# rmazzier/OpenSetGaitRecognition_PCAA

Hardware: AMD Instinct MI355X
Metric: gait sequences/sec (train step) (higher is better)
Workload: dtype bf16; 1 GPU; PCAA V4 train step (enc+dec+disc fwd/bwd, WGAN-GP, Chamfer, 2x Adam), B=64/GPU T=30 N=128 C=4 K=8, BASELINE config[1]; global_batch=64, precision=bf16, parallelism=dp1, sync_bn=False, finite_loss=True, hip_graph=False, decoder_update=fused wgrad+adam

## Files before the change

include/pcaa_hip.h:

```cpp
#ifndef PCAA_HIP_H
#define PCAA_HIP_H

#include <stddef.h>

#ifdef __cplusplus
extern "C" {
#endif

#define PCAA_ABI_VERSION 20

#define PCAA_OK 0
#define PCAA_ERR_INVALID_ARG 1
#define PCAA_ERR_LAUNCH 2

#define PCAA_F32 0
#define PCAA_BF16 1
#define PCAA_SPLIT_F16 2

#define PCAA_LAYOUT_KC 0
#define PCAA_LAYOUT_RC 1

#define PCAA_ACT_NONE 0
#define PCAA_ACT_ELU 1

const char* pcaa_last_error(void);
int pcaa_abi_version(void);

int pcaa_gemm(int math,
              const void* A, int a_dtype, int a_layout, long lda,
              const void* B, int b_dtype, int b_layout, long ldb,
              void* C, int c_dtype, long ldc,
              int M, int N, int K,
              const float* bias, double* colstats, int nrep,
              int split_k, int accumulate, void* stream);

int pcaa_gemm_num_splits(int math, int K, int split_k);
int pcaa_gemm_group_rc_f32(int n, const void* const* A, const void* const* B, void* const* C, const int* M,
                           const int* N, const int* K, const int* split_k, void* stream);
int pcaa_gemm_group_rc_f32_slabs(int n, const void* const* A, const void* const* B, void* const* slabs, const int* M,
                                 const int* N, const int* K, const int* split_k, void* stream);
int pcaa_gemm_v2_enable(int on);
int pcaa_gemm_slabs(int math,
                    const void* A, int a_dtype, int a_layout, long lda,
                    const void* B, int b_dtype, int b_layout, long ldb,
                    float* slabs, long slab_stride, int M, int N, int K, int split_k, void* stream);
int pcaa_gemm_affine_elu(const void* A, long lda, const void* W, long ldw, void* out, long ldo,
                         const float* scale, const float* shift, int M, int N, int K, int pool_rows,
                         void* stream);
int pcaa_gemm_dgrad_bn_supported(int M, int N, int K);
int pcaa_gemm_dgrad_bn(const void* dy, long lddy, const void* Wt, long ldw, const void* y, void* dz, long ld,
                       const float* scale, const float* shift, const float* mean, const float* rstd,
                       double* stats, int nrep, int M, int N, int K,
                       const float* x, int xc, const float* W1, void* stream);
int pcaa_bn_bwd_dy_split(const float* dz, const float* y, void* dy_img, const float* coef, long rows, int ch,
                         float img_scale, void* stream);
int pcaa_gemm_dgrad_bn_split3(const void* dy_img, long lddy, const void* Wt_img, long ldw, const float* y, float* dz,
                              long ld, const float* scale, const float* shift, const float* mean, const float* rstd,
                              double* stats, int nrep, int M, int N, int K, float out_scale, void* stream);
int pcaa_timing_events_create(void** start, void** stop);
int pcaa_timing_events_destroy(void* start, void* stop);
int pcaa_time_next_gemm(void* start, void* stop);
int pcaa_timing_pending(void);
int pcaa_timing_elapsed_ms(void* start, void* stop, float* ms);
int pcaa_splitk_reduce(const float* slabs, int nsplit, long slab_stride, long n, float* out,
                       int accumulate, void* stream);
int pcaa_splitk_reduce_stats(const float* slabs, int nsplit, long slab_stride, float* out,
                             double* stats, int nrep, long rows, int ch, void* stream);

int pcaa_pointnet_in_fwd(const float* x, int C, const float* W, const float* bias, void* y, int y_dtype,
                         long P, int cout, double* stats, int nrep, void* stream);
int pcaa_pointnet_in_wgrad(const void* dy, int dy_dtype, const float* x, int C, float* dW, long P,
                           int cout, void* stream);
int pcaa_pointnet_in_apply(const float* x, int C, const float* W, const float* scale, const float* shift,
                           void* a, int a_dtype, long P, int cout, void* stream);
int pcaa_pointnet_in_bwd_stats(const void* da, int dtype, const float* x, int C, const float* W,
                               const float* scale, const float* shift, const float* mean, const float* rstd,
                               double* stats, int nrep, long P, int cout, void* stream);
int pcaa_pointnet_in_bwd_onepass(const void* da, int dtype, const float* x, int C, const float* W,
                                 const float* scale, const float* shift, const float* mean, const float* rstd,
                                 double* stats, int nrep, float* G, long P, int cout, const double* pivot_mom,
                                 double pivot_inv_count, void* stream);
int pcaa_pointnet_in_bwd_onepass_rows(const void* da, int dtype, const float* x, int C, const float* W,
                                      const float* scale, const float* shift, const float* mean, const float* rstd,
                                      double* stats, int nrep, float* G, long P, int cout, const double* pivot_mom,
                                      double pivot_inv_count, void* stream);
int pcaa_pointnet_in_bwd_g_rows(long P);
int pcaa_points_moments_size(void);
int pcaa_points_moments(const float* x, int C, long P, double* mom, void* stream);
int pcaa_pointnet_in_bwd_combine(const float* G, int nrep, const float* W, const double* mom, const float* coef,
                                 float* dW, int cout, int C, long P, const double* pivot_mom, double pivot_inv_count,
                                 void* stream);
int pcaa_pointnet_in_moment_stats(const double* mom, const float* W, int C, int cout, void* stream);
int pcaa_pointnet_in_bwd_wgrad(const void* da, int dtype, const float* x, int C, const float* W,
                               const float* scale, const float* shift, const float* coef, float* dW,
                               long P, int cout, int dz_is_pre ,
                               void* stream);

int pcaa_cast_bf16(const float* src, void* dst, void* dst_t, int R, int C, void* stream);

int pcaa_bn_finalize(const double* stats, int nrep, long count, const float* lin_bias,
                     const float* gamma, const float* beta,
                     float* running_mean, float* running_var, long long* num_batches_tracked,
                     float momentum, float eps,
                     float* scale, float* shift, float* mean, float* rstd, int ch, void* stream);
int pcaa_bn_eval_coeffs(const float* gamma, const float* beta, const float* running_mean,
                        const float* running_var, const float* lin_bias, float eps, float* scale,
                        float* shift, int ch, void* stream);
int pcaa_bn_act_fwd(const void* y, void* a, int dtype, const float* scale, const float* shift,
                    long rows, int ch, void* stream);
int pcaa_bn_act_meanpool_fwd(const void* y, int dtype, const float* scale, const float* shift,
                             const float* mean, const float* rstd, float* pooled, float* e1, float* e2,
                             long groups, int group_rows, int ch, void* stream);
int pcaa_bn_pool_bwd_stats(const float* dpool, const float* e1, const float* e2, float pool_scale,
                           double* stats, int nrep, long groups, int ch, void* stream);
int pcaa_bn_act_bwd_dz(const void* da, const float* dpool, int group_rows, float pool_scale,
                       const void* y, void* dz, int dtype,
                       const float* scale, const float* shift, const float* mean, const float* rstd,
                       double* stats, int nrep, long rows, int ch, void* stream);
int pcaa_bn_bwd_finalize(const double* stats, int nrep, long count, const float* gamma,
                         const float* mean, const float* rstd,
                         float* coef, float* dgamma, float* dbeta, int ch, void* stream);
int pcaa_bn_bwd_dy(const void* dz, const void* y, void* dy, int dtype, const float* coef,
                   long rows, int ch, void* stream);
int pcaa_bn_tail_arm_fwd(const double* stats, int nrep, long count, const float* lin_bias,
                         const float* gamma, const float* beta,
                         float* running_mean, float* running_var, long long* num_batches_tracked,
                         float momentum, float eps,
                         float* scale, float* shift, float* mean, float* rstd, int ch, unsigned* counter);
int pcaa_bn_tail_arm_bwd(const double* stats, int nrep, long count, const float* gamma,
                         const float* mean, const float* rstd,
                         float* coef, float* dgamma, float* dbeta, int ch, unsigned* counter);
int pcaa_bn_tail_pending(void);
int pcaa_bn_tail_disarm(void);
int pcaa_bn_bwd_dy_fused(const void* da, const float* dpool, int group_rows, float pool_scale,
                         const void* y, void* dy, int dtype, const float* scale, const float* shift,
                         const float* coef, long rows, int ch, void* stream);

int pcaa_bias_act(float* y, const float* bias, int act, long rows, int cols, void* stream);
int pcaa_elu_bwd_from_out(const float* da, const float* a, float* dz, long n, void* stream);
int pcaa_colsum(const float* x, float* out, long rows, int cols, void* stream);
int pcaa_sum(const float* x, long n, float scale, float* out, void* stream);
int pcaa_rowsum(const float* x, float* out, long rows, int cols, float scale, void* stream);
int pcaa_scale_by_device_scalar(const float* x, const float* s, float* out, long n, void* stream);
int pcaa_scale_rows(const float* x, const float* s, float* out, long rows, int cols, void* stream);
int pcaa_prior_sample(const float* z0, const float* means, const long long* gt, int B, int K, int D,
                      float* z, float* onehot, void* stream);
int pcaa_pack_points(const float* src, long sb, long sc, long st, long sn,
                     float* dst, int B, int C, int T, int N, void* stream);

int pcaa_gather_rows(const void* src, long n_src_rows, long row_bytes, const long long* idx, void* dst,
                     long n_rows, int* err_flag, void* stream);

int pcaa_dtc_im2col(const float* a, float* col, int B, int T, int Cin, int dilation, void* stream);
int pcaa_dtc_col2im(const float* dcol, float* da, int B, int T, int Cin, int dilation, void* stream);

int pcaa_chamfer_fwd_bwd(const float* preds, long p_sb, long p_sc, long p_st, long p_sn,
                         const float* gts, long g_sb, long g_sc, long g_st, long g_sn,
                         int B, int T, int N, int C, float* frame_loss,
                         float* dpreds, long d_sb, long d_sc, long d_st, long d_sn,
                         float grad_scale, const float* grad_per_b, void* stream);
int pcaa_cross_entropy(const float* logits, const long long* target, int B, int K,
                       float* loss, float* dlogits, float grad_scale, long long* preds,
                       int* err_flag, void* stream);

int pcaa_disc_forward(const float* x, const float* label, int B, int K,
                      const float* W1, const float* b1, const float* W2, const float* b2,
                      const float* W3, const float* b3, float* out, void* stream);
int pcaa_disc_backward(const float* x, const float* label, int B, int K,
                       const float* W1, const float* b1, const float* W2, const float* b2,
                       const float* W3, const float* b3, const float* gout,
                       float* dx, float* dlabel,
                       float* dW1, float* db1, float* dW2, float* db2, float* dW3, float* db3,
                       float* workspace, size_t workspace_bytes, void* stream);
int pcaa_disc_backward_backward(const float* x, const float* label, int B, int K,
                                const float* W1, const float* b1, const float* W2, const float* b2,
                                const float* W3, const float* b3, const float* gout, const float* gbar,
                                float* dx2, float* dlabel2, float* dgout,
                                float* dW1, float* db1, float* dW2, float* db2, float* dW3, float* db3,
                                float* workspace, size_t workspace_bytes, void* stream);
size_t pcaa_disc_workspace_bytes(int B, int K);
int pcaa_disc_wgan_gp(const float* z, const float* fv, const float* label, const float* alphas,
                      int B, int K,
                      const float* W1, const float* b1, const float* W2, const float* b2,
                      const float* W3, const float* b3, float gp_weight, float* losses,
                      float* dW1, float* db1, float* dW2, float* db2, float* dW3, float* db3,
                      float* dz, float* workspace, size_t workspace_bytes, void* stream);

int pcaa_joint_likelihood(const float* x, const float* means, int B, int K, int D, double* lik,
                          void* stream);
int pcaa_kvote(const double* lik, const long long* preds, double threshold, int k, int n_labels,
               int n_classes, int n_windows, long long* out, void* stream);

int pcaa_skinny_supported(int M, int N, int K);
int pcaa_skinny_splits(int kind, int M, int N, int K);
int pcaa_skinny_linear_fwd(const float* x, long ldx, const float* W, long ldw, const float* bias, int act,
                           float* y, float* ws, long ws_floats, int M, int N, int K, int nsplit,
                           void* stream);
int pcaa_skinny_linear_dgrad(const float* dz, long lddz, const float* W, long ldw, float* dx,
                             const float* a_prev, int accumulate, float* ws, long ws_floats, int M, int N,
                             int K, int nsplit, void* stream);
int pcaa_skinny_linear_wgrad(const float* dz, long lddz, const float* x, long ldx, float* dW, long lddw,
                             int M, int N, int K, void* stream);
int pcaa_skinny_linear_fwd_exact(const float* x, long ldx, const float* W, long ldw, const float* bias, int act,
                                 float* y, float* ws, long ws_floats, int M, int N, int K, int nsplit, void* stream);
int pcaa_skinny_linear_dgrad_exact(const float* dz, long lddz, const float* W, long ldw, float* dx,
                                   const float* a_prev, int accumulate, float* ws, long ws_floats, int M, int N,
                                   int K, int nsplit, void* stream);
int pcaa_skinny_linear_wgrad_exact(const float* dz, long lddz, const float* x, long ldx, float* dW, long lddw,
                                   int M, int N, int K, void* stream);
int pcaa_skinny_linear_wgrad_adam_exact(const float* dz, long lddz, const float* x, long ldx, float* W,
                                        float* exp_avg, float* exp_avg_sq, long ldw, int M, int N, int K,
                                        float beta1, float beta2, float eps, float grad_scale,
                                        const float* coef_dev, void* stream);
int pcaa_skinny_linear_wgrad_bf16(const float* dz, long lddz, const float* x, long ldx, void* dW_bf16, long lddw,
                                  int M, int N, int K, void* stream);
int pcaa_skinny_linear_wgrad_adam(const float* dz, long lddz, const float* x, long ldx, float* W,
                                  float* exp_avg, float* exp_avg_sq, long ldw, int M, int N, int K,
                                  float beta1, float beta2, float eps, float grad_scale,
                                  const float* coef_dev, void* stream);
int pcaa_skinny_linear_wgrad_adam_rows(const float* dz, long lddz, const float* x, long ldx, float* W,
                                       float* exp_avg, float* exp_avg_sq, long ldw, int M, int N, int K,
                                       float beta1, float beta2, float eps, float grad_scale,
                                       const float* coef_dev, int rows_alloc, void* stream);
long pcaa_packed_chunk_elems(int N, int K);
int pcaa_pack_rows_t16(const float* dz, long lddz, int N, const float* x, long ldx, int K, int rows, void* chunk_bf16,
                       void* stream);
int pcaa_skinny_linear_wgrad_adam_t16(const void* packed_bf16, long chunk_stride, int chunks, float* W, float* exp_avg,
                                      float* exp_avg_sq, long ldw, int N, int K, float beta1, float beta2, float eps,
                                      float grad_scale, const float* coef_dev, void* stream);
int pcaa_skinny_linear_fwd_w16(const float* x, long ldx, const void* W16, long ldw, const float* bias, int act,
                               float* y, float* ws, long ws_floats, int M, int N, int K, int nsplit, void* stream);
int pcaa_skinny_linear_dgrad_w16(const float* dz, long lddz, const void* W16, long ldw, float* dx,
                                 const float* a_prev, int accumulate, float* ws, long ws_floats, int M, int N,
                                 int K, int nsplit, void* stream);

int pcaa_dtc_conv_supported(int T, int cin, int cout);
int pcaa_dtc_conv_ksplit(int B, int cin, int cout);
int pcaa_dtc_conv_fwd(const float* src, const float* scale, const float* shift, const float* W, float* y,
                      float* col, double* stats, int nrep, int B, int T, int cin, int cout, int dilation,
                      int ksplit, long slab_stride, void* stream);
int pcaa_dtc_conv_fwd_bf16(const float* src, const float* scale, const float* shift, const float* W, float* y,
                      float* col, double* stats, int nrep, int B, int T, int cin, int cout, int dilation,
                      int ksplit, long slab_stride, void* stream);
// ... 4 lines not shown
                          void* stream);
int pcaa_dtc_conv_fwd_win_bf16(const float* table, const float* scale, const float* shift, const float* W, float* y,
                          float* col, double* stats, int nrep, int B, int T, int cin, int cout, int dilation,
                          int ksplit, long slab_stride, const int* win_row, long table_rows, long ring_rows,
                          void* stream);

int pcaa_dtc_conv_fwd_seg(const float* table, const float* scale, const float* shift, const float* W, float* y,
                          int B, int T, int cin, int cout, int dilation, int ksplit, long slab_stride,
                          const int* win_row, long n_seg, long ring_rows, void* stream);
int pcaa_dtc_conv_fwd_seg_bf16(const float* table, const float* scale, const float* shift, const float* W, float* y,
                          int B, int T, int cin, int cout, int dilation, int ksplit, long slab_stride,
                          const int* win_row, long n_seg, long ring_rows, void* stream);

int pcaa_crop_overlap_vec_bytes(const float* crops, long crop_elems, long frame_elems);
int pcaa_crop_overlap(const float* crops, long crop_elems, long frame_elems, int M, int T, int hop, int* same,
                      void* stream);
int pcaa_gather_rows_w4(const void* src, long n_src_rows, long row_words, const long long* idx, void* dst,
                        long n_rows, int* err_flag, void* stream);

int pcaa_scatter_rows(const void* src, const int* dst_row, long n_rows, long row_words, void* dst, long n_dst_rows,
                      int* err_flag, void* stream);
int pcaa_stream_score(const float* logits, const float* sup_fv, const float* means, const int* run_start, int n_runs,
                      const int* win_stream, const int* win_j, const int* vote_pos, int nw, int K, int D, int Kc,
                      double threshold, int k, int n_labels, int n_classes, double* hist_lik, long long* hist_pred,
                      int max_streams, long long* preds, double* lik, long long* votes, int n_votes, void* stream);

#define PCAA_RAW_MAX_CARD 1024
#define PCAA_RAW_MAX_POINTS 1024
int pcaa_frames_from_raw(const void* points, int points_f64, long P, const int* offsets, int n, const int* pick,
                         const int* frame_key, long seed, int N, int C, int standardize, int divide_by_std,
                         float* out, int n_out, int* pick_out, int* err_flag, void* stream);
int pcaa_dtc_conv_dgrad_ksplit(int B, int cin, int cout);
int pcaa_dtc_conv_dgrad(const float* dy, const float* dz, const float* y, const float* coef, float* dy_out,
                        const float* W, float* out, const float* ep_y, const float* ep_scale,
                        const float* ep_shift, const float* ep_mean, const float* ep_rstd, double* ep_stats,
                        int nrep, int B, int T, int cin, int cout, int dilation, int ksplit, long slab_stride,
                        void* stream);
int pcaa_dtc_conv_dgrad_bf16(const float* dy, const float* dz, const float* y, const float* coef, float* dy_out,
                        const float* W, float* out, const float* ep_y, const float* ep_scale,
                        const float* ep_shift, const float* ep_mean, const float* ep_rstd, double* ep_stats,
                        int nrep, int B, int T, int cin, int cout, int dilation, int ksplit, long slab_stride,
                        void* stream);

int pcaa_heads_supported(int B, int K, int d_in, int d_sup, int d_head, int d_proj, int backward);
int pcaa_heads_fwd(const float* x4, const float* W1, const float* b1, const float* Wh, const float* bh,
                   const float* W2, const float* b2, const float* Wg, const float* bg, float* sup_fv,
                   float* h, float* logits, float* hproj, int B, int K, void* stream);
int pcaa_heads_bwd(const float* x4, const float* sup_fv, const float* h, const float* logits,
                   const float* hproj, const float* W1, const float* Wh, const float* W2,
                   const float* Wg, const float* d_logits, const float* d_sup, const float* d_hproj,
                   float* dW1, float* db1, float* dWh, float* dbh, float* dW2, float* db2, float* dWg,
                   float* dbg, float* dx4, int B, int K, void* stream);

int pcaa_gemm_split3_supported(int M, int N, int K);
int pcaa_gemm_split3(const void* A, const void* B, int layout, long lda, long ldb, float* C, long ldc, int M,
                     int N, int K, double* colstats, int nrep, float out_scale, void* stream);
int pcaa_gemm_split3_num_splits(int K, int split_k);
int pcaa_gemm_slabs_split3(const void* A, const void* B, int layout, long lda, long ldb, float* slabs,
                           long slab_stride, int M, int N, int K, int split_k, float out_scale, void* stream);
int pcaa_split_f16(const float* src, void* dst_img, long rows, int ch, int transpose, float img_scale, void* stream);
int pcaa_set_range_flag(int* dev_flag);
int pcaa_bn_act_fwd_split(const float* y, void* a_img, const float* scale, const float* shift, long rows,
                          int ch, float img_scale, void* stream);
int pcaa_bn_bwd_dy_fused_split(const float* da, const float* dpool, int group_rows, float pool_scale,
                               const float* y, void* dy_img, const float* scale, const float* shift,
                               const float* coef, long rows, int ch, float img_scale, void* stream);

int pcaa_orced_heads_supported(int B, int K, int d_in, int d_lat);
int pcaa_orced_heads_fwd(const float* x4, const float* Wmu, const float* bmu, const float* Wlv, const float* blv,
                         const float* eps, const float* Wc, const float* bc, float* mu, float* logvar, float* sup_fv,
                         float* logits, int B, int K, int d_in, int d_lat, void* stream);
int pcaa_orced_heads_bwd(const float* x4, const float* eps, const float* logvar, const float* sup_fv,
                         const float* Wmu, const float* Wlv, const float* Wc, const float* d_logits,
                         const float* d_sup, const float* d_mu, const float* d_logvar, float* ws, float* dWmu,
                         float* dbmu, float* dWlv, float* dblv, float* dWc, float* dbc, float* dx4, int B, int K,
                         int d_in, int d_lat, void* stream);
int pcaa_orced_kl(const float* mu, const float* logvar, const float* mu_k, float* loss, float* d_mu,
                  float* d_logvar, float* d_muk, float gscale, int B, int d_lat, void* stream);

int pcaa_adam_step(float* param, const float* grad, float* exp_avg, float* exp_avg_sq, long n,
                   float lr, float beta1, float beta2, float eps, int step, float grad_scale,
                   int max_blocks, void* stream);
int pcaa_adam_advance(int* step_dev, float* coef_dev, float lr, float beta1, float beta2, void* stream);
int pcaa_adam_step_dev(float* param, const float* grad, float* exp_avg, float* exp_avg_sq, long n,
                       float beta1, float beta2, float eps, const float* coef_dev, float grad_scale,
                       int max_blocks, void* stream);
int pcaa_adam_step_dev_g16(float* param, const void* grad_bf16, float* exp_avg, float* exp_avg_sq, long n,
                           float beta1, float beta2, float eps, const float* coef_dev, float grad_scale,
                           int max_blocks, void* stream);

#ifdef __cplusplus
}
#endif
#endif
```

opensetgaitrecognition_pcaa_amd/csrc/elementwise.hip:

```cpp
#include <stdarg.h>

#include "common.h"
#include "bn_tail.h"

static thread_local char g_err[512] = "";
void pcaa_set_error(const char* fmt, ...) {
  va_list ap;
  va_start(ap, fmt);
  vsnprintf(g_err, sizeof(g_err), fmt, ap);
  va_end(ap);
}
extern "C" const char* pcaa_last_error(void) { return g_err; }
static thread_local int* g_range_flag = nullptr;
int* pcaa_range_flag_ptr() { return g_range_flag; }
extern "C" int pcaa_set_range_flag(int* dev_flag) { g_range_flag = dev_flag; return PCAA_OK; }
extern "C" int pcaa_abi_version(void) { return PCAA_ABI_VERSION; }

namespace {

constexpr int ROWS_PER_BLOCK = 128;

inline bool ch_ok(int ch) {
  if (ch < 4 || ch > 1024 || (ch & 3)) return false;
  const int q = ch >> 2;
// ... 455 lines not shown
    const int n = (int)(r % N); r /= N;
    const int t = (int)(r % T);
    const long b = r / T;
    dst[i] = src[b * sb + c * sc + t * st + n * sn];
  }
}

__global__ void dtc_im2col_kernel(const float* __restrict__ a, float* __restrict__ col, int B, int T,
                                  int Cin, int d) {
  const long total = (long)B * T * Cin * 3;
  for (long i = (long)blockIdx.x * blockDim.x + threadIdx.x; i < total; i += (long)gridDim.x * blockDim.x) {
    const int tap = (int)(i % 3);
    long r = i / 3;
    const int ci = (int)(r % Cin); r /= Cin;
    const int t = (int)(r % T);
    const long b = r / T;
    const int ts = t - (2 - tap) * d;
    col[i] = ts >= 0 ? a[(b * T + ts) * Cin + ci] : 0.f;
  }
}

__global__ void dtc_col2im_kernel(const float* __restrict__ dcol, float* __restrict__ da, int B, int T,
                                  int Cin, int d) {
  const long total = (long)B * T * Cin;
  for (long i = (long)blockIdx.x * blockDim.x + threadIdx.x; i < total; i += (long)gridDim.x * blockDim.x) {
    const int ci = (int)(i % Cin);
    long r = i / Cin;
    const int t = (int)(r % T);
    const long b = r / T;
    float acc = 0.f;
#pragma unroll
    for (int tap = 0; tap < 3; ++tap) {
      const int tt = t + (2 - tap) * d;
      if (tt < T) acc += dcol[((b * T + tt) * Cin + ci) * 3 + tap];
    }
    da[i] = acc;
  }
}

template <int U, typename TG = float>
__global__ __launch_bounds__(256) void adam_kernel(float* __restrict__ p, const TG* __restrict__ g,
                                                   float* __restrict__ m, float* __restrict__ v, long n,
                                                   float b1, float b2, float eps, float step_size,
                                                   float inv_bc2_sqrt, float grad_scale,
                                                   const float* __restrict__ coef) {
  if (coef) {
    step_size = coef[0];
    inv_bc2_sqrt = coef[1];
  }
  const long nq = n >> 2;
  const long stride = (long)gridDim.x * 256;
  for (long q0 = (long)blockIdx.x * 256 + threadIdx.x; q0 < nq; q0 += stride * U) {
    f32x4 pv[U], gv[U], mv[U], vv[U];
#pragma unroll
    for (int u = 0; u < U; ++u) {
      const long q = q0 + u * stride;
      if (q < nq) { pv[u] = load4(p + q * 4); gv[u] = load4(g + q * 4); mv[u] = load4(m + q * 4); vv[u] = load4(v + q * 4); }
    }
#pragma unroll
    for (int u = 0; u < U; ++u) {
      const long q = q0 + u * stride;
      if (q >= nq) break;
#pragma unroll
      for (int e = 0; e < 4; ++e) {
        float pe = pv[u][e], me = mv[u][e], ve = vv[u][e];
        adam_update(pe, me, ve, gv[u][e] * grad_scale, b1, b2, eps, step_size, inv_bc2_sqrt);
        pv[u][e] = pe; mv[u][e] = me; vv[u][e] = ve;
      }
      store4(p + q * 4, pv[u]);
      store4(m + q * 4, mv[u]);
      store4(v + q * 4, vv[u]);
    }
  }
  if (blockIdx.x == 0 && threadIdx.x < (n & 3)) {
    const long i = (nq << 2) + threadIdx.x;
    float pp = p[i], mm = m[i], vv = v[i];
    adam_update(pp, mm, vv, (float)g[i] * grad_scale, b1, b2, eps, step_size, inv_bc2_sqrt);
    m[i] = mm;
    v[i] = vv;
    p[i] = pp;
  }
}

__global__ void adam_coef_kernel(int* __restrict__ step, float* __restrict__ coef, float lr, float b1, float b2) {
  const int t = *step + 1;
  *step = t;
  const double bc1 = 1.0 - pow((double)b1, (double)t);
  const double bc2 = 1.0 - pow((double)b2, (double)t);
  coef[0] = (float)((double)lr / bc1);
  coef[1] = (float)(1.0 / sqrt(bc2));
}

inline int grid_for(long work_items, int per_block = 256, int cap = 256 * 8) {
  long g = cdiv(work_items, per_block);
  if (g < 1) g = 1;
  if (g > cap) g = cap;
  return (int)g;
}

inline int col_invariant_grid(long nquads, int qpr) {
  int a = qpr, b = 256;
  while (b) { const int t = a % b; a = b; b = t; }
  const int unit = qpr / a;
  long g = cdiv(nquads, 256);
  if (g > 2048) g = 2048;
  g = cdiv(g, unit) * unit;
  return (int)g;
}

}

extern "C" int pcaa_bn_finalize(const double* stats, int nrep, long count, const float* lin_bias,
                                const float* gamma, const float* beta, float* running_mean,
                                float* running_var, long long* num_batches_tracked, float momentum,
                                float eps, float* scale, float* shift, float* mean, float* rstd,
                                int ch, void* stream) {
  PCAA_CHECK_ARG(stats && gamma && beta && scale && shift && mean && rstd, "pcaa_bn_finalize: null pointer");
  PCAA_CHECK_ARG(nrep >= 1 && count >= 1 && ch >= 1, "pcaa_bn_finalize: bad sizes");
  PCAA_CHECK_ARG((running_mean == nullptr) == (running_var == nullptr), "pcaa_bn_finalize: running stats must come together");
  const double unbias = count > 1 ? (double)count / (double)(count - 1) : 1.0;
  hipLaunchKernelGGL(bn_finalize_kernel, dim3((unsigned)cdiv(ch, 256)), dim3(256), 0, as_stream(stream),
                     stats, nrep, 1.0 / (double)count, unbias, lin_bias, gamma, beta, running_mean,
                     running_var, num_batches_tracked, momentum, eps, scale, shift, mean, rstd, ch);
  PCAA_RETURN_LAUNCH_STATUS("pcaa_bn_finalize");
}

extern "C" int pcaa_bn_eval_coeffs(const float* gamma, const float* beta, const float* running_mean,
                                   const float* running_var, const float* lin_bias, float eps, float* scale,
                                   float* shift, int ch, void* stream) {
  PCAA_CHECK_ARG(gamma && beta && running_mean && running_var && scale && shift && ch >= 1, "pcaa_bn_eval_coeffs: bad args");
  hipLaunchKernelGGL(bn_eval_coeffs_kernel, dim3((unsigned)cdiv(ch, 256)), dim3(256), 0, as_stream(stream),
                     gamma, beta, running_mean, running_var, lin_bias, eps, scale, shift, ch);
  PCAA_RETURN_LAUNCH_STATUS("pcaa_bn_eval_coeffs");
}

extern "C" int pcaa_bn_act_fwd(const void* y, void* a, int dtype, const float* scale, const float* shift,
                               long rows, int ch, void* stream) {
  PCAA_CHECK_ARG(y && a && scale && shift, "pcaa_bn_act_fwd: null pointer");
  PCAA_CHECK_ARG(rows >= 1 && ch >= 4 && (ch & 3) == 0, "pcaa_bn_act_fwd: ch must be a multiple of 4");
  const long nq = rows * (ch >> 2);
  PCAA_CHECK_ARG(nq < (1L << 31), "pcaa_bn_act_fwd: tensor too large for 32-bit quad indices");
  const int grid = col_invariant_grid(nq, ch >> 2);
  if (dtype == PCAA_F32)
    hipLaunchKernelGGL(bn_act_fwd_kernel<float>, dim3(grid), dim3(256), 0, as_stream(stream),
                       (const float*)y, (float*)a, scale, shift, (unsigned)nq, (unsigned)(ch >> 2));
  else if (dtype == PCAA_BF16)
    hipLaunchKernelGGL(bn_act_fwd_kernel<bf16_t>, dim3(grid), dim3(256), 0, as_stream(stream),
                       (const bf16_t*)y, (bf16_t*)a, scale, shift, (unsigned)nq, (unsigned)(ch >> 2));
  else { pcaa_set_error("pcaa_bn_act_fwd: bad dtype"); return PCAA_ERR_INVALID_ARG; }
  PCAA_RETURN_LAUNCH_STATUS("pcaa_bn_act_fwd");
}

extern "C" int pcaa_bn_act_fwd_split(const float* y, void* a_img, const float* scale, const float* shift, long rows,
                                     int ch, float img_scale, void* stream) {
  PCAA_CHECK_ARG(y && a_img && scale && shift, "pcaa_bn_act_fwd_split: null pointer");
  PCAA_CHECK_ARG(rows >= 1 && ch >= 4 && (ch & 3) == 0, "pcaa_bn_act_fwd_split: ch must be a multiple of 4");
  const long nq = rows * (ch >> 2);
  PCAA_CHECK_ARG(nq < (1L << 31), "pcaa_bn_act_fwd_split: tensor too large for 32-bit quad indices");
  const int grid = col_invariant_grid(nq, ch >> 2);
  hipLaunchKernelGGL(bn_act_fwd_split_kernel, dim3(grid), dim3(256), 0, as_stream(stream), y, (split_t*)a_img, scale, shift,
                     (unsigned)nq, (unsigned)(ch >> 2), img_scale, pcaa_range_flag_ptr());
  PCAA_RETURN_LAUNCH_STATUS("pcaa_bn_act_fwd_split");
}

extern "C" int pcaa_split_f16(const float* src, void* dst_img, long rows, int ch, int transpose, float img_scale,
                               void* stream) {
  PCAA_CHECK_ARG(src && dst_img && rows >= 1 && ch >= 1, "pcaa_split_f16: bad args");
  long g = cdiv(rows * ch, 256);
  if (g > 4096) g = 4096;
  hipLaunchKernelGGL(split_f16_kernel, dim3((unsigned)g), dim3(256), 0, as_stream(stream), src, (split_t*)dst_img, rows, ch,
                     transpose, img_scale, pcaa_range_flag_ptr());
  PCAA_RETURN_LAUNCH_STATUS("pcaa_split_f16");
}
// ... 303 lines not shown
  const int n = B * (D > K ? D : K);
  hipLaunchKernelGGL(prior_sample_kernel, dim3((unsigned)cdiv(n, 256)), dim3(256), 0, as_stream(stream), z0, means, gt, B, K, D, z, onehot);
  PCAA_RETURN_LAUNCH_STATUS("pcaa_prior_sample");
}

extern "C" int pcaa_pack_points(const float* src, long sb, long sc, long st, long sn, float* dst,
                                int B, int C, int T, int N, void* stream) {
  PCAA_CHECK_ARG(src && dst && B >= 1 && C >= 1 && T >= 1 && N >= 1, "pcaa_pack_points: bad args");
  const long n = (long)B * C * T * N;
  hipLaunchKernelGGL(pack_points_kernel, dim3(grid_for(n)), dim3(256), 0, as_stream(stream), src, sb, sc, st, sn, dst, B, C, T, N);
  PCAA_RETURN_LAUNCH_STATUS("pcaa_pack_points");
}

namespace {
__global__ __launch_bounds__(256) void gather_rows_kernel(const uint4* __restrict__ src, const long long* __restrict__ idx,
                                                          long n_src, uint4* __restrict__ dst, long n_rows,
                                                          long row_vec, int* __restrict__ err) {
  const long total = n_rows * row_vec;
  for (long v = (long)blockIdx.x * 256 + threadIdx.x; v < total; v += (long)gridDim.x * 256) {
    const long r = v / row_vec, off = v - r * row_vec;
    const long long i = idx[r];
    uint4 val = {0u, 0u, 0u, 0u};
    if (i >= 0 && i < n_src) val = src[i * row_vec + off];
    else if (err != nullptr && off == 0) atomicOr(err, 1);
    dst[v] = val;
  }
}
}

extern "C" int pcaa_gather_rows(const void* src, long n_src_rows, long row_bytes, const long long* idx, void* dst,
                                long n_rows, int* err_flag, void* stream) {
  PCAA_CHECK_ARG(src && idx && dst && n_src_rows >= 1 && n_rows >= 1 && row_bytes >= 16 && row_bytes % 16 == 0,
                 "pcaa_gather_rows: bad args (rows are multiples of 16 bytes)");
  PCAA_CHECK_ARG(((uintptr_t)src % 16) == 0 && ((uintptr_t)dst % 16) == 0, "pcaa_gather_rows: 16-B alignment");
  const long row_vec = row_bytes / 16;
  hipLaunchKernelGGL(gather_rows_kernel, dim3(grid_for(n_rows * row_vec, 256, 256 * 16)), dim3(256), 0, as_stream(stream),
                     reinterpret_cast<const uint4*>(src), idx, n_src_rows, reinterpret_cast<uint4*>(dst), n_rows,
                     row_vec, err_flag);
  PCAA_RETURN_LAUNCH_STATUS("pcaa_gather_rows");
}

extern "C" int pcaa_dtc_im2col(const float* a, float* col, int B, int T, int Cin, int dilation, void* stream) {
  PCAA_CHECK_ARG(a && col && B >= 1 && T >= 1 && Cin >= 1 && dilation >= 1, "pcaa_dtc_im2col: bad args");
  const long n = (long)B * T * Cin * 3;
  hipLaunchKernelGGL(dtc_im2col_kernel, dim3(grid_for(n)), dim3(256), 0, as_stream(stream), a, col, B, T, Cin, dilation);
  PCAA_RETURN_LAUNCH_STATUS("pcaa_dtc_im2col");
}

extern "C" int pcaa_dtc_col2im(const float* dcol, float* da, int B, int T, int Cin, int dilation, void* stream) {
  PCAA_CHECK_ARG(dcol && da && B >= 1 && T >= 1 && Cin >= 1 && dilation >= 1, "pcaa_dtc_col2im: bad args");
  const long n = (long)B * T * Cin;
  hipLaunchKernelGGL(dtc_col2im_kernel, dim3(grid_for(n)), dim3(256), 0, as_stream(stream), dcol, da, B, T, Cin, dilation);
  PCAA_RETURN_LAUNCH_STATUS("pcaa_dtc_col2im");
}

namespace {
__device__ __forceinline__ void slab_sum(const float* __restrict__ base, int nsplit, long stride, f32x4& acc) {
  int s = 0;
  for (; s + 8 <= nsplit; s += 8) {
    f32x4 v[8];
#pragma unroll
    for (int u = 0; u < 8; ++u) v[u] = load4(base + (s + u) * stride);
#pragma unroll
    for (int u = 0; u < 8; ++u) acc += v[u];
  }
  for (; s < nsplit; ++s) acc += load4(base + s * stride);
}

__global__ __launch_bounds__(256) void splitk_reduce_kernel(const float* __restrict__ slabs, int nsplit,
                                                            long stride, long nquads, float* __restrict__ out,
                                                            int accumulate) {
  for (long q = (long)blockIdx.x * 256 + threadIdx.x; q < nquads; q += (long)gridDim.x * 256) {
    f32x4 acc = accumulate ? load4(out + q * 4) : f32x4{0.f, 0.f, 0.f, 0.f};
    slab_sum(slabs + q * 4, nsplit, stride, acc);
    store4(out + q * 4, acc);
  }
}
}

namespace {
__global__ __launch_bounds__(256) void splitk_reduce_stats_kernel(const float* __restrict__ slabs, int nsplit,
                                                                  long stride, float* __restrict__ out,
                                                                  double* __restrict__ stats, int nrep,
                                                                  long rows, int ch) {
  __shared__ f32x4 red[2][256];
  const int qpr = ch >> 2, rl = 256 / qpr;
  const int cq = threadIdx.x % qpr, rlane = threadIdx.x / qpr;
  const int c = cq * 4;
  constexpr int RPB = 32;
  const long r0 = (long)blockIdx.x * RPB, r1 = min(rows, r0 + RPB);
  f32x4 s1 = {0.f, 0.f, 0.f, 0.f}, s2 = {0.f, 0.f, 0.f, 0.f};
  for (long r = r0 + rlane; r < r1; r += rl) {
    f32x4 acc = {0.f, 0.f, 0.f, 0.f};
    slab_sum(slabs + r * ch + c, nsplit, stride, acc);
    store4(out + r * ch + c, acc);
    s1 += acc;
    s2 += acc * acc;
  }
  red[0][threadIdx.x] = s1;
  red[1][threadIdx.x] = s2;
  __syncthreads();
  for (int o = threadIdx.x; o < 2 * ch; o += 256) {
    const int stat = o / ch, cc = o - stat * ch;
    double v = 0.0;
    for (int l = 0; l < rl; ++l) v += (double)red[stat][l * qpr + (cc >> 2)][cc & 3];
    unsafeAtomicAdd(&stats[((long)(blockIdx.x % nrep) * 2 + stat) * ch + cc], v);
  }
}
}

extern "C" int pcaa_splitk_reduce_stats(const float* slabs, int nsplit, long slab_stride, float* out,
                                        double* stats, int nrep, long rows, int ch, void* stream) {
  PCAA_CHECK_ARG(slabs && out && stats && nsplit >= 1 && nrep >= 1 && rows >= 1, "pcaa_splitk_reduce_stats: bad args");
  PCAA_CHECK_ARG(ch_ok(ch) && (slab_stride % 4) == 0, "pcaa_splitk_reduce_stats: ch/4 must divide 256 (ch=%d)", ch);
  hipLaunchKernelGGL(splitk_reduce_stats_kernel, dim3((unsigned)cdiv(rows, 32)), dim3(256), 0, as_stream(stream),
                     slabs, nsplit, slab_stride, out, stats, nrep, rows, ch);
  PCAA_RETURN_LAUNCH_STATUS("pcaa_splitk_reduce_stats");
}

extern "C" int pcaa_splitk_reduce(const float* slabs, int nsplit, long slab_stride, long n, float* out,
                                  int accumulate, void* stream) {
  PCAA_CHECK_ARG(slabs && out && nsplit >= 1 && n >= 4 && (n % 4) == 0 && (slab_stride % 4) == 0,
                 "pcaa_splitk_reduce: n and slab_stride must be multiples of 4");
  PCAA_CHECK_ARG(((uintptr_t)slabs % 16) == 0 && ((uintptr_t)out % 16) == 0, "pcaa_splitk_reduce: 16-B alignment");
  hipLaunchKernelGGL(splitk_reduce_kernel, dim3(grid_for(n >> 2)), dim3(256), 0, as_stream(stream), slabs, nsplit,
                     slab_stride, n >> 2, out, accumulate);
  PCAA_RETURN_LAUNCH_STATUS("pcaa_splitk_reduce");
}

static int launch_adam(float* param, const float* grad, float* exp_avg, float* exp_avg_sq, long n, float beta1,
                       float beta2, float eps, float step_size, float inv_bc2_sqrt, const float* coef,
                       float grad_scale, int max_blocks, void* stream, const char* what) {
  PCAA_CHECK_ARG(((uintptr_t)param % 16) == 0 && ((uintptr_t)grad % 16) == 0 && ((uintptr_t)exp_avg % 16) == 0 &&
                 ((uintptr_t)exp_avg_sq % 16) == 0, "pcaa_adam_step: buffers must be 16-B aligned");
  const int cap = max_blocks > 0 ? max_blocks : 256 * 16;
  if (cap <= 1024)
    hipLaunchKernelGGL(adam_kernel<4>, dim3(grid_for(n >> 4, 256, cap)), dim3(256), 0, as_stream(stream), param, grad,
                       exp_avg, exp_avg_sq, n, beta1, beta2, eps, step_size, inv_bc2_sqrt, grad_scale, coef);
  else
    hipLaunchKernelGGL(adam_kernel<1>, dim3(grid_for(n >> 2, 256, cap)), dim3(256), 0, as_stream(stream), param, grad,
                       exp_avg, exp_avg_sq, n, beta1, beta2, eps, step_size, inv_bc2_sqrt, grad_scale, coef);
  PCAA_RETURN_LAUNCH_STATUS(what);
}

extern "C" int pcaa_adam_step_dev_g16(float* param, const void* grad_bf16, float* exp_avg, float* exp_avg_sq, long n,
                                      float beta1, float beta2, float eps, const float* coef_dev, float grad_scale,
                                      int max_blocks, void* stream) {
  PCAA_CHECK_ARG(param && grad_bf16 && exp_avg && exp_avg_sq && coef_dev && n >= 1 && max_blocks >= 0,
                 "pcaa_adam_step_dev_g16: bad args");
  PCAA_CHECK_ARG(((uintptr_t)param % 16) == 0 && ((uintptr_t)grad_bf16 % 8) == 0 && ((uintptr_t)exp_avg % 16) == 0 &&
                 ((uintptr_t)exp_avg_sq % 16) == 0, "pcaa_adam_step_dev_g16: buffers must be 16-B (gradient: 8-B) aligned");
  const bf16_t* g = reinterpret_cast<const bf16_t*>(grad_bf16);
  const int cap = max_blocks > 0 ? max_blocks : 256 * 16;
  if (cap <= 1024)
    hipLaunchKernelGGL((adam_kernel<4, bf16_t>), dim3(grid_for(n >> 4, 256, cap)), dim3(256), 0, as_stream(stream), param, g,
                       exp_avg, exp_avg_sq, n, beta1, beta2, eps, 0.f, 0.f, grad_scale, coef_dev);
  else
    hipLaunchKernelGGL((adam_kernel<1, bf16_t>), dim3(grid_for(n >> 2, 256, cap)), dim3(256), 0, as_stream(stream), param, g,
                       exp_avg, exp_avg_sq, n, beta1, beta2, eps, 0.f, 0.f, grad_scale, coef_dev);
  PCAA_RETURN_LAUNCH_STATUS("pcaa_adam_step_dev_g16");
}

extern "C" int pcaa_adam_step(float* param, const float* grad, float* exp_avg, float* exp_avg_sq, long n,
                              float lr, float beta1, float beta2, float eps, int step, float grad_scale,
                              int max_blocks, void* stream) {
  PCAA_CHECK_ARG(param && grad && exp_avg && exp_avg_sq && n >= 1 && step >= 1 && max_blocks >= 0,
                 "pcaa_adam_step: bad args");
  const double bc1 = 1.0 - pow((double)beta1, (double)step);
  const double bc2 = 1.0 - pow((double)beta2, (double)step);
  return launch_adam(param, grad, exp_avg, exp_avg_sq, n, beta1, beta2, eps, (float)((double)lr / bc1),
                     (float)(1.0 / sqrt(bc2)), nullptr, grad_scale, max_blocks, stream, "pcaa_adam_step");
}

extern "C" int pcaa_adam_advance(int* step_dev, float* coef_dev, float lr, float beta1, float beta2, void* stream) {
  PCAA_CHECK_ARG(step_dev && coef_dev, "pcaa_adam_advance: bad args");
  hipLaunchKernelGGL(adam_coef_kernel, dim3(1), dim3(1), 0, as_stream(stream), step_dev, coef_dev, lr, beta1, beta2);
  PCAA_RETURN_LAUNCH_STATUS("pcaa_adam_advance");
}

extern "C" int pcaa_adam_step_dev(float* param, const float* grad, float* exp_avg, float* exp_avg_sq, long n,
                                  float beta1, float beta2, float eps, const float* coef_dev, float grad_scale,
                                  int max_blocks, void* stream) {
  PCAA_CHECK_ARG(param && grad && exp_avg && exp_avg_sq && coef_dev && n >= 1 && max_blocks >= 0,
                 "pcaa_adam_step_dev: bad args");
  return launch_adam(param, grad, exp_avg, exp_avg_sq, n, beta1, beta2, eps, 0.f, 0.f, coef_dev, grad_scale,
                     max_blocks, stream, "pcaa_adam_step_dev");
}
```

opensetgaitrecognition_pcaa_amd/csrc/losses.hip:

```cpp
#include "common.h"

namespace {

constexpr int MAXC = 8;
constexpr int CH_THREADS = 256;

__global__ __launch_bounds__(CH_THREADS) void chamfer_kernel(
    const float* __restrict__ preds, long p_sb, long p_sc, long p_st, long p_sn,
    const float* __restrict__ gts, long g_sb, long g_sc, long g_st, long g_sn,
    int T, int N, int C, float* __restrict__ frame_loss,
    float* __restrict__ dpreds, long d_sb, long d_sc, long d_st, long d_sn,
    float grad_scale, const float* __restrict__ grad_per_b) {
  extern __shared__ __attribute__((aligned(16))) float sm[];
  float* sg = sm;
  float* sp = sg + (long)N * MAXC;
  float* rg = sp + (long)N * MAXC;
  float* rp = rg + N;
  int* nn = reinterpret_cast<int*>(rp + N);
  __shared__ float red[CH_THREADS / 64];

  const int frame = blockIdx.x;
  const int b = frame / T, t = frame - b * T;
  const float* pb = preds + b * p_sb + t * p_st;
  const float* gb = gts + b * g_sb + t * g_st;

  for (int e = threadIdx.x; e < N * MAXC; e += CH_THREADS) {
    const int n = e / MAXC, c = e - n * MAXC;
    sg[e] = (c < C) ? gb[c * g_sc + n * g_sn] : 0.f;
    sp[e] = (c < C) ? pb[c * p_sc + n * p_sn] : 0.f;
  }
  __syncthreads();
  for (int n = threadIdx.x; n < N; n += CH_THREADS) {
    float a = 0.f, q = 0.f;
#pragma unroll
    for (int c = 0; c < MAXC; ++c) {
      a = fmaf(sg[n * MAXC + c], sg[n * MAXC + c], a);
      q = fmaf(sp[n * MAXC + c], sp[n * MAXC + c], q);
    }
    rg[n] = a;
    rp[n] = q;
  }
  __syncthreads();

  const float w = grad_scale * (grad_per_b ? grad_per_b[b] : 1.f);
  float loss = 0.f;
  for (int item = threadIdx.x; item < 2 * N; item += CH_THREADS) {
    const bool dir1 = item < N;
    const int me = dir1 ? item : item - N;
    const float* mine = dir1 ? sp : sg;
    const float* other = dir1 ? sg : sp;
    const float* rother = dir1 ? rg : rp;
    float v[MAXC];
#pragma unroll
    for (int c = 0; c < MAXC; ++c) v[c] = mine[me * MAXC + c];
    const float rme = dir1 ? rp[me] : rg[me];
    float best = 3.4e38f;
    int bi = 0;
    for (int o = 0; o < N; ++o) {
      float dot = 0.f;
#pragma unroll
      for (int c = 0; c < MAXC; ++c) dot = fmaf(other[o * MAXC + c], v[c], dot);
      const float P = (dir1 ? (rother[o] + rme) : (rme + rother[o])) - 2.f * dot;
      if (P < best) { best = P; bi = o; }
    }
    loss += best;
    nn[item] = bi;
  }
  loss = wave_sum(loss);
  if ((threadIdx.x & 63) == 0) red[threadIdx.x >> 6] = loss;
  __syncthreads();
  if (threadIdx.x == 0) {
    float tot = 0.f;
    for (int i = 0; i < CH_THREADS / 64; ++i) tot += red[i];
    frame_loss[frame] = tot;
  }
  if (dpreds) {
    __syncthreads();
    float* db = dpreds + b * d_sb + t * d_st;
    for (int e = threadIdx.x; e < N * C; e += CH_THREADS) {
      const int c = e / N, n = e - c * N;
      const float pv = sp[n * MAXC + c];
      float g = 2.f * w * (pv - sg[nn[n] * MAXC + c]);
      for (int i = 0; i < N; ++i)
        if (nn[N + i] == n) g += 2.f * w * (pv - sg[i * MAXC + c]);
      db[c * d_sc + n * d_sn] = g;
    }
  }
}

__global__ __launch_bounds__(256) void cross_entropy_kernel(const float* __restrict__ logits,
                                                            const long long* __restrict__ target, int B,
                                                            int K, float* loss, float* dlogits,
                                                            float grad_scale, long long* preds, int* err_flag) {
  __shared__ double red[4];
  double acc = 0.0;
  for (int r = threadIdx.x; r < B; r += 256) {
    const float* x = logits + (long)r * K;
    float mx = x[0];
    for (int k = 1; k < K; ++k) mx = fmaxf(mx, x[k]);
    float se = 0.f;
    for (int k = 0; k < K; ++k) se += expf(x[k] - mx);
    const float inv = 1.f / se;
    int am = 0;
    float pbest = -1.f;
    long long tg = target ? target[r] : 0;
    if (tg < 0 || tg >= K) {
      if (err_flag) *err_flag = 1;
      tg = 0;
    }
    for (int k = 0; k < K; ++k) {
      const float pk = expf(x[k] - mx) / se;
      if (pk > pbest) { pbest = pk; am = k; }
      if (dlogits) dlogits[(long)r * K + k] = grad_scale * (expf(x[k] - mx) * inv - (k == tg ? 1.f : 0.f)) / (float)B;
    }
    if (preds) preds[r] = am;
    if (target) acc += (double)(logf(se) + mx - x[tg]);
  }
  acc = wave_sum_d(acc);
  if ((threadIdx.x & 63) == 0) red[threadIdx.x >> 6] = acc;
  __syncthreads();
  if (threadIdx.x == 0 && loss) loss[0] = (float)((red[0] + red[1] + red[2] + red[3]) / B);
}

}

extern "C" int pcaa_chamfer_fwd_bwd(const float* preds, long p_sb, long p_sc, long p_st, long p_sn,
                                    const float* gts, long g_sb, long g_sc, long g_st, long g_sn,
                                    int B, int T, int N, int C, float* frame_loss, float* dpreds,
                                    long d_sb, long d_sc, long d_st, long d_sn, float grad_scale,
                                    const float* grad_per_b, void* stream) {
  PCAA_CHECK_ARG(preds && gts && frame_loss, "pcaa_chamfer_fwd_bwd: null pointer");
  PCAA_CHECK_ARG(B >= 1 && T >= 1 && N >= 1 && C >= 1 && C <= MAXC, "pcaa_chamfer_fwd_bwd: need 1<=C<=%d (C=%d)", MAXC, C);
  const size_t lds = ((size_t)2 * N * MAXC + 4 * (size_t)N) * sizeof(float);
  PCAA_CHECK_ARG(lds <= 150 * 1024, "pcaa_chamfer_fwd_bwd: N=%d too large for one LDS tile", N);
  if (lds > 64 * 1024) {
    hipError_t e = hipFuncSetAttribute(reinterpret_cast<const void*>(chamfer_kernel),
                                       hipFuncAttributeMaxDynamicSharedMemorySize, (int)lds);
    if (e != hipSuccess) { pcaa_set_error("pcaa_chamfer_fwd_bwd: cannot raise LDS limit: %s", hipGetErrorString(e)); return PCAA_ERR_LAUNCH; }
  }
  hipLaunchKernelGGL(chamfer_kernel, dim3((unsigned)(B * T)), dim3(CH_THREADS), lds, as_stream(stream),
                     preds, p_sb, p_sc, p_st, p_sn, gts, g_sb, g_sc, g_st, g_sn, T, N, C, frame_loss,
                     dpreds, d_sb, d_sc, d_st, d_sn, grad_scale, grad_per_b);
  PCAA_RETURN_LAUNCH_STATUS("pcaa_chamfer_fwd_bwd");
}

extern "C" int pcaa_cross_entropy(const float* logits, const long long* target, int B, int K, float* loss,
                                  float* dlogits, float grad_scale, long long* preds, int* err_flag,
                                  void* stream) {
  PCAA_CHECK_ARG(logits && B >= 1 && K >= 1, "pcaa_cross_entropy: bad args");
  PCAA_CHECK_ARG(target || (!loss && !dlogits), "pcaa_cross_entropy: loss/grad need targets");
  hipLaunchKernelGGL(cross_entropy_kernel, dim3(1), dim3(256), 0, as_stream(stream), logits, target, B, K,
                     loss, dlogits, grad_scale, preds, err_flag);
  PCAA_RETURN_LAUNCH_STATUS("pcaa_cross_entropy");
}
```

opensetgaitrecognition_pcaa_amd/csrc/pointnet_in.hip:

```cpp
#include "common.h"
#include "bn_tail.h"

namespace {

constexpr int MAXC = 8;
constexpr int FWD_ROWS = 128;
constexpr int WG_ROWS = 256;
constexpr int BWD_ROWS = 256;

template <typename T, int CP>
__global__ __launch_bounds__(256) void pointnet_in_fwd_kernel(const float* __restrict__ x, int C,
                                                              const float* __restrict__ W,
                                                              const float* __restrict__ bias,
                                                              T* __restrict__ y, long P, int cout,
                                                              double* __restrict__ stats, int nrep, BnTail tail) {
  __shared__ float xs[FWD_ROWS * CP];
  __shared__ f32x4 red[2][256];
  __shared__ int tail_flag;
  typedef float f32x2 __attribute__((ext_vector_type(2)));
  const int qpr = cout >> 2, rl = 256 / qpr;
  const int cq = threadIdx.x % qpr, rlane = threadIdx.x / qpr;
  const long r0 = (long)blockIdx.x * FWD_ROWS;
  const int nrows = (int)min((long)FWD_ROWS, P - r0);
  for (int e = threadIdx.x; e < FWD_ROWS * CP; e += 256) {
// ... 269 lines not shown
    if (MODE == 3) __syncthreads();
  }
  if (MODE != 0) {
    float* red = xs;
#pragma unroll
    for (int j = 0; j < 4; ++j)
#pragma unroll
      for (int c = 0; c < CP; ++c) red[(rlane * cout + cq * 4 + j) * CP + c] = acc[j][c];
    __syncthreads();
    for (int o = threadIdx.x; o < cout * C; o += 256) {
      const int ch = o / C, c = o - ch * C;
      float v = 0.f;
      for (int l = 0; l < rl; ++l) v += red[(l * cout + ch) * CP + c];
      if (MODE == 3 && g_row_per_wg) dW[(long)blockIdx.x * cout * C + o] = v;
      else atomicAdd(&dW[(MODE == 3 ? (long)(blockIdx.x % nrep) * cout * C : 0L) + o], v);
    }
  }
  if (MODE == 0 || MODE == 3) bn_tail_run(tail, threadIdx.x, 256, gridDim.x, &tail_flag);
}

template <int CP>
__global__ __launch_bounds__(256) void points_moments_kernel(const float* __restrict__ x, int C, long P,
                                                             double* __restrict__ mom) {
  constexpr int NV = CP * (CP + 1) / 2 + CP;
  __shared__ double red[4][NV];
  double a[NV];
#pragma unroll
  for (int i = 0; i < NV; ++i) a[i] = 0.0;
  for (long r = (long)blockIdx.x * 256 + threadIdx.x; r < P; r += (long)gridDim.x * 256) {
    double xv[CP];
    if (CP == 4 && C == 4) {
      const f32x4 v = load4(x + r * 4);
      xv[0] = v.x; xv[1] = v.y; xv[2] = v.z; xv[3] = v.w;
    } else {
#pragma unroll
      for (int c = 0; c < CP; ++c) xv[c] = c < C ? (double)x[r * C + c] : 0.0;
    }
    int i = 0;
#pragma unroll
    for (int k = 0; k < CP; ++k)
#pragma unroll
      for (int c = k; c < CP; ++c) { a[i] = fma(xv[k], xv[c], a[i]); ++i; }
#pragma unroll
    for (int c = 0; c < CP; ++c) a[i + c] += xv[c];
  }
#pragma unroll
  for (int i = 0; i < NV; ++i) {
    const double v = wave_sum_d(a[i]);
    if ((threadIdx.x & 63) == 0) red[threadIdx.x >> 6][i] = v;
  }
  __syncthreads();
  if (threadIdx.x < NV) {
    const double v = red[0][threadIdx.x] + red[1][threadIdx.x] + red[2][threadIdx.x] + red[3][threadIdx.x];
    int i = threadIdx.x;
    if (i < CP * (CP + 1) / 2) {
      int k = 0;
      while (i >= CP - k) { i -= CP - k; ++k; }
      const int c = k + i;
      unsafeAtomicAdd(&mom[k * MAXC + c], v);
      if (c != k) unsafeAtomicAdd(&mom[c * MAXC + k], v);
    } else {
      unsafeAtomicAdd(&mom[MAXC * MAXC + (i - CP * (CP + 1) / 2)], v);
    }
  }
}

__global__ void pointnet_in_moment_stats_kernel(const double* __restrict__ mom, const float* __restrict__ W, int C,
                                                BnTail t) {
  const int o = blockIdx.x * blockDim.x + threadIdx.x;
  if (o == 0 && t.kind == 1 && t.nbt != nullptr) *t.nbt += 1;
  if (o >= t.ch) return;
  double w[MAXC];
  for (int k = 0; k < MAXC; ++k) w[k] = k < C ? (double)W[o * C + k] : 0.0;
  double s1 = 0.0, s2 = 0.0;
  for (int k = 0; k < C; ++k) {
    s1 += w[k] * mom[MAXC * MAXC + k];
    double row = 0.0;
    for (int c = 0; c < C; ++c) row += mom[k * MAXC + c] * w[c];
    s2 += w[k] * row;
  }
  bn_tail_channel(t, o, s1, s2);
}

__global__ __launch_bounds__(256) void pointnet_in_bwd_combine_kernel(const float* __restrict__ G, int g_rows,
                                                                      const float* __restrict__ W,
                                                                      const double* __restrict__ mom,
                                                                      const float* __restrict__ coef,
                                                                      float* __restrict__ dW, int cout, int C, double P,
                                                                      const double* __restrict__ pivot_mom,
                                                                      double pivot_inv_count) {
  __shared__ double red[4];
  const int i = blockIdx.x;
  const int o = i / C, c = i - o * C;
  double g = 0.0;
  for (int r = threadIdx.x; r < g_rows; r += 256) g += (double)G[(long)r * cout * C + i];
  g = wave_sum_d(g);
  if ((threadIdx.x & 63) == 0) red[threadIdx.x >> 6] = g;
  __syncthreads();
  if (threadIdx.x != 0) return;
  g = (red[0] + red[1]) + (red[2] + red[3]);
  const double piv = pivot_mom ? (double)(float)(pivot_mom[MAXC * MAXC + c] * pivot_inv_count) : 0.0;
  double yx = 0.0;
  for (int k = 0; k < C; ++k) yx += (double)W[o * C + k] * (mom[k * MAXC + c] - piv * mom[MAXC * MAXC + k]);
  dW[i] = (float)((double)coef[o] * g + (double)coef[cout + o] * yx +
                  (double)coef[2 * cout + o] * (mom[MAXC * MAXC + c] - P * piv));
}

template <typename T>
__global__ __launch_bounds__(256) void pointnet_in_wgrad_kernel(const T* __restrict__ dy,
                                                                const float* __restrict__ x, int C,
                                                                float* __restrict__ dW, long P, int cout) {
  __shared__ float xs[(WG_ROWS * MAXC > 8192) ? WG_ROWS * MAXC : 8192];
  const int qpr = cout >> 2, rl = 256 / qpr;
  const int cq = threadIdx.x % qpr, rlane = threadIdx.x / qpr;
  const long r0 = (long)blockIdx.x * WG_ROWS;
  const int nrows = (int)min((long)WG_ROWS, P - r0);
  for (int e = threadIdx.x; e < WG_ROWS * MAXC; e += 256) {
    const int r = e / MAXC, c = e - r * MAXC;
    xs[e] = (r < nrows && c < C) ? x[(r0 + r) * C + c] : 0.f;
  }
  __syncthreads();
  float acc[4][MAXC];
#pragma unroll
  for (int j = 0; j < 4; ++j)
#pragma unroll
    for (int c = 0; c < MAXC; ++c) acc[j][c] = 0.f;
  int r = rlane;
  for (; r + 3 * rl < nrows; r += 4 * rl) {
    f32x4 d[4];
#pragma unroll
    for (int u = 0; u < 4; ++u) d[u] = load4(dy + (r0 + r + u * rl) * cout + cq * 4);
#pragma unroll
    for (int u = 0; u < 4; ++u) {
#pragma unroll
      for (int c = 0; c < MAXC; ++c) {
        const float xv = xs[(r + u * rl) * MAXC + c];
        acc[0][c] = fmaf(d[u].x, xv, acc[0][c]);
        acc[1][c] = fmaf(d[u].y, xv, acc[1][c]);
        acc[2][c] = fmaf(d[u].z, xv, acc[2][c]);
        acc[3][c] = fmaf(d[u].w, xv, acc[3][c]);
      }
    }
  }
  for (; r < nrows; r += rl) {
    const f32x4 d = load4(dy + (r0 + r) * cout + cq * 4);
#pragma unroll
    for (int c = 0; c < MAXC; ++c) {
      const float xv = xs[r * MAXC + c];
      acc[0][c] = fmaf(d.x, xv, acc[0][c]);
      acc[1][c] = fmaf(d.y, xv, acc[1][c]);
      acc[2][c] = fmaf(d.z, xv, acc[2][c]);
      acc[3][c] = fmaf(d.w, xv, acc[3][c]);
    }
  }
  __syncthreads();
  float* red = xs;
#pragma unroll
  for (int j = 0; j < 4; ++j)
#pragma unroll
    for (int c = 0; c < MAXC; ++c) red[(rlane * cout + cq * 4 + j) * MAXC + c] = acc[j][c];
  __syncthreads();
  for (int o = threadIdx.x; o < cout * C; o += 256) {
    const int ch = o / C, c = o - ch * C;
    float v = 0.f;
    for (int l = 0; l < rl; ++l) v += red[(l * cout + ch) * MAXC + c];
    atomicAdd(&dW[o], v);
// ... 87 lines not shown
extern "C" int pcaa_pointnet_in_bwd_stats(const void* da, int dtype, const float* x, int C, const float* W,
                                          const float* scale, const float* shift, const float* mean,
                                          const float* rstd, double* stats, int nrep, long P, int cout,
                                          void* stream) {
  PCAA_CHECK_ARG(da && x && W && scale && shift && mean && rstd && stats && P >= 1 && nrep >= 1,
                 "pcaa_pointnet_in_bwd_stats: bad args");
  PCAA_CHECK_ARG(shape_ok(C, cout), "pcaa_pointnet_in_bwd_stats: need C<=%d and cout/4 dividing 256 (C=%d cout=%d)", MAXC, C, cout);
  const unsigned grid = (unsigned)cdiv(P, BWD_ROWS);
  const BnTail tail = pcaa_take_bn_tail(stats);
  if (dtype == PCAA_F32)
    LAUNCH_BWD(float, 0, (const float*)da, x, C, W, scale, shift, mean, rstd, nullptr, stats, nrep, nullptr, P, cout, tail);
  else if (dtype == PCAA_BF16)
    LAUNCH_BWD(bf16_t, 0, (const bf16_t*)da, x, C, W, scale, shift, mean, rstd, nullptr, stats, nrep, nullptr, P, cout, tail);
  else { pcaa_set_error("pcaa_pointnet_in_bwd_stats: bad dtype"); return PCAA_ERR_INVALID_ARG; }
  PCAA_RETURN_LAUNCH_STATUS("pcaa_pointnet_in_bwd_stats");
}

extern "C" int pcaa_pointnet_in_bwd_wgrad(const void* da, int dtype, const float* x, int C, const float* W,
                                          const float* scale, const float* shift, const float* coef, float* dW,
                                          long P, int cout, int dz_is_pre, void* stream) {
  PCAA_CHECK_ARG(da && x && W && scale && shift && coef && dW && P >= 1, "pcaa_pointnet_in_bwd_wgrad: bad args");
  PCAA_CHECK_ARG(shape_ok(C, cout), "pcaa_pointnet_in_bwd_wgrad: need C<=%d and cout/4 dividing 256 (C=%d cout=%d)", MAXC, C, cout);
  const unsigned grid = (unsigned)cdiv(P, BWD_ROWS);
  if (dtype == PCAA_F32 && !dz_is_pre)
    LAUNCH_BWD(float, 1, (const float*)da, x, C, W, scale, shift, nullptr, nullptr, coef, nullptr, 1, dW, P, cout, BnTail{});
  else if (dtype == PCAA_F32)
    LAUNCH_BWD(float, 2, (const float*)da, x, C, W, scale, shift, nullptr, nullptr, coef, nullptr, 1, dW, P, cout, BnTail{});
  else if (dtype == PCAA_BF16 && !dz_is_pre)
    LAUNCH_BWD(bf16_t, 1, (const bf16_t*)da, x, C, W, scale, shift, nullptr, nullptr, coef, nullptr, 1, dW, P, cout, BnTail{});
  else if (dtype == PCAA_BF16)
    LAUNCH_BWD(bf16_t, 2, (const bf16_t*)da, x, C, W, scale, shift, nullptr, nullptr, coef, nullptr, 1, dW, P, cout, BnTail{});
  else { pcaa_set_error("pcaa_pointnet_in_bwd_wgrad: bad dtype"); return PCAA_ERR_INVALID_ARG; }
  PCAA_RETURN_LAUNCH_STATUS("pcaa_pointnet_in_bwd_wgrad");
}

static int pointnet_in_bwd_onepass(const void* da, int dtype, const float* x, int C, const float* W, const float* scale,
                                   const float* shift, const float* mean, const float* rstd, double* stats, int nrep,
                                   float* G, long P, int cout, const double* pivot_mom, double pivot_inv_count,
                                   int g_row_per_wg, void* stream) {
  PCAA_CHECK_ARG(da && x && W && scale && shift && mean && rstd && stats && G && P >= 1 && nrep >= 1,
                 "pcaa_pointnet_in_bwd_onepass: bad args");
  PCAA_CHECK_ARG(shape_ok(C, cout), "pcaa_pointnet_in_bwd_onepass: need C<=%d and cout/4 dividing 256 (C=%d cout=%d)", MAXC, C, cout);
  const unsigned grid = (unsigned)cdiv(P, BWD_ROWS);
  const BnTail tail = pcaa_take_bn_tail(stats);
  if (dtype == PCAA_F32)
    LAUNCH_BWD(float, 3, (const float*)da, x, C, W, scale, shift, mean, rstd, nullptr, stats, nrep, G, P, cout, tail,
               pivot_mom, pivot_inv_count, g_row_per_wg);
  else if (dtype == PCAA_BF16)
    LAUNCH_BWD(bf16_t, 3, (const bf16_t*)da, x, C, W, scale, shift, mean, rstd, nullptr, stats, nrep, G, P, cout, tail,
               pivot_mom, pivot_inv_count, g_row_per_wg);
  else { pcaa_set_error("pcaa_pointnet_in_bwd_onepass: bad dtype"); return PCAA_ERR_INVALID_ARG; }
  PCAA_RETURN_LAUNCH_STATUS("pcaa_pointnet_in_bwd_onepass");
}

extern "C" int pcaa_pointnet_in_bwd_onepass(const void* da, int dtype, const float* x, int C, const float* W,
                                            const float* scale, const float* shift, const float* mean,
                                            const float* rstd, double* stats, int nrep, float* G, long P, int cout,
                                            const double* pivot_mom, double pivot_inv_count, void* stream) {
  return pointnet_in_bwd_onepass(da, dtype, x, C, W, scale, shift, mean, rstd, stats, nrep, G, P, cout, pivot_mom,
                                 pivot_inv_count, 0, stream);
}

extern "C" int pcaa_pointnet_in_bwd_onepass_rows(const void* da, int dtype, const float* x, int C, const float* W,
                                                 const float* scale, const float* shift, const float* mean,
                                                 const float* rstd, double* stats, int nrep, float* G, long P, int cout,
                                                 const double* pivot_mom, double pivot_inv_count, void* stream) {
  return pointnet_in_bwd_onepass(da, dtype, x, C, W, scale, shift, mean, rstd, stats, nrep, G, P, cout, pivot_mom,
                                 pivot_inv_count, 1, stream);
}

extern "C" int pcaa_pointnet_in_bwd_g_rows(long P) { return (int)cdiv(P, BWD_ROWS); }

extern "C" int pcaa_points_moments_size(void) { return MAXC * MAXC + MAXC; }

extern "C" int pcaa_points_moments(const float* x, int C, long P, double* mom, void* stream) {
  PCAA_CHECK_ARG(x && mom && C >= 1 && C <= MAXC && P >= 1, "pcaa_points_moments: bad args");
  long g = cdiv(P, 256 * 4);
  if (g > 512) g = 512;
  if (C <= 4) hipLaunchKernelGGL(points_moments_kernel<4>, dim3((unsigned)g), dim3(256), 0, as_stream(stream), x, C, P, mom);
  else hipLaunchKernelGGL(points_moments_kernel<8>, dim3((unsigned)g), dim3(256), 0, as_stream(stream), x, C, P, mom);
  PCAA_RETURN_LAUNCH_STATUS("pcaa_points_moments");
}

extern "C" int pcaa_pointnet_in_moment_stats(const double* mom, const float* W, int C, int cout, void* stream) {
  PCAA_CHECK_ARG(mom && W && C >= 1 && C <= MAXC && cout >= 1, "pcaa_pointnet_in_moment_stats: bad args");
  const BnTail t = pcaa_take_bn_tail(mom);
  PCAA_CHECK_ARG(t.kind == 1 && t.ch == cout, "pcaa_pointnet_in_moment_stats: arm the forward finalize on `mom` first "
                 "(pcaa_bn_tail_arm_fwd)");
  hipLaunchKernelGGL(pointnet_in_moment_stats_kernel, dim3((unsigned)cdiv(cout, 256)), dim3(256), 0, as_stream(stream), mom,
                     W, C, t);
  PCAA_RETURN_LAUNCH_STATUS("pcaa_pointnet_in_moment_stats");
}

extern "C" int pcaa_pointnet_in_bwd_combine(const float* G, int nrep, const float* W, const double* mom,
                                            const float* coef, float* dW, int cout, int C, long P,
                                            const double* pivot_mom, double pivot_inv_count, void* stream) {
  PCAA_CHECK_ARG(G && W && mom && coef && dW && cout >= 1 && C >= 1 && C <= MAXC && nrep >= 1,
                 "pcaa_pointnet_in_bwd_combine: bad args");
  hipLaunchKernelGGL(pointnet_in_bwd_combine_kernel, dim3((unsigned)(cout * C)), dim3(256), 0,
                     as_stream(stream), G, nrep, W, mom, coef, dW, cout, C, (double)P, pivot_mom, pivot_inv_count);
  PCAA_RETURN_LAUNCH_STATUS("pcaa_pointnet_in_bwd_combine");
}

extern "C" int pcaa_cast_bf16(const float* src, void* dst, void* dst_t, int R, int C, void* stream) {
  PCAA_CHECK_ARG(src && (dst || dst_t) && R >= 1 && C >= 1, "pcaa_cast_bf16: bad args");
  const long n = (long)R * C;
  long g = cdiv(n, 256);
  if (g > 2048) g = 2048;
  hipLaunchKernelGGL(cast_bf16_kernel, dim3((unsigned)g), dim3(256), 0, as_stream(stream), src, (bf16_t*)dst,
                     (bf16_t*)dst_t, R, C);
  PCAA_RETURN_LAUNCH_STATUS("pcaa_cast_bf16");
}
```

opensetgaitrecognition_pcaa_amd/ops.py:

```python
import ctypes
import os

import torch

from . import _lib
from ._lib import ACT_ELU, ACT_NONE, KC, PCAA_BF16, PCAA_F32, RC, check

PCAA_SPLIT_F16 = 2

NREP = 16
BN_EPS = 1e-5
BN_MOMENTUM = 0.1


def _p(t):
    return None if t is None else t.data_ptr()


_raw_stream = getattr(torch._C, "_cuda_getCurrentRawStream", None)
_raw_device = getattr(torch._C, "_cuda_getDevice", None)


def _s():
    if _raw_stream is not None and _raw_device is not None:
# ... 70 lines not shown
        return self.only_prefix is None or key.startswith(self.only_prefix)

    def summary(self):
        torch.cuda.synchronize()
        agg = {}
        for key, flops, nbytes, ev in self.records:
            if not ev.valid():
                continue
            a = agg.setdefault(key, {"launches": 0, "ms": 0.0, "flops": 0.0, "bytes": 0.0})
            a["launches"] += 1
            a["ms"] += ev.elapsed_ms()
            a["flops"] += flops
            a["bytes"] += nbytes
        return agg


class _TorchEvents:

    def __init__(self):
        self.e0 = torch.cuda.Event(enable_timing=True)
        self.e1 = torch.cuda.Event(enable_timing=True)
        self.e0.record()

    def end(self):
        self.e1.record()
        return self

    def valid(self):
        return True

    def elapsed_ms(self):
        return self.e0.elapsed_time(self.e1)


class _KernelEvents:

    def __init__(self):
        lib = _lib.load()
        self.a, self.b = ctypes.c_void_p(), ctypes.c_void_p()
        check(lib.pcaa_timing_events_create(ctypes.byref(self.a), ctypes.byref(self.b)), "pcaa_timing_events_create")
        check(lib.pcaa_time_next_gemm(self.a, self.b), "pcaa_time_next_gemm")
        self.ok = False

    def end(self):
        lib = _lib.load()
        self.ok = not lib.pcaa_timing_pending()
        if not self.ok:
            lib.pcaa_time_next_gemm(None, None)
        return self

    def valid(self):
        return self.ok

    def elapsed_ms(self):
        ms = ctypes.c_float()
        check(_lib.load().pcaa_timing_elapsed_ms(self.a, self.b, ctypes.byref(ms)), "pcaa_timing_elapsed_ms")
        return float(ms.value)

    def __del__(self):
        try:
            _lib.load().pcaa_timing_events_destroy(self.a, self.b)
        except Exception:
            pass


def _begin_timing(key):
    return _KernelEvents() if key.startswith(("gemm_bf16_v2_kernel", "gemm_bf16_v2rc_kernel")) else _TorchEvents()


TIMER = None


def set_timer(timer):
    global TIMER
    TIMER = timer


class StatsPool:

    def __init__(self, device, capacity_doubles=4 << 20):
        self.buf = torch.zeros(capacity_doubles, dtype=torch.float64, device=device)
        self.off = 0

    def begin(self):
        if self.off:
            self.buf[:self.off].zero_()
        self.off = 0

    def take_raw(self, n):
        n = (n + 1) // 2 * 2
        if self.off + n > self.buf.numel():
            return None
        v = self.buf[self.off:self.off + n]
        self.off += n
        return v

    def take(self, ch):
        n = NREP * 2 * ch
        if self.off + n + 2 > self.buf.numel():
            return None
        v = self.buf[self.off:self.off + n].view(NREP, 2, ch)
        v._pcaa_counter = self.buf[self.off + n:self.off + n + 1].view(torch.int32)
        self.off += n + 2
        return v


STATS_POOL = None


def set_stats_pool(pool):
    global STATS_POOL
    STATS_POOL = pool


def new_stats(ch, device):
    if STATS_POOL is not None and STATS_POOL.buf.device == torch.device(device):
        v = STATS_POOL.take(ch)
        if v is not None:
            return v
    buf = torch.zeros(NREP * 2 * ch + 2, dtype=torch.float64, device=device)
    v = buf[:NREP * 2 * ch].view(NREP, 2, ch)
    v._pcaa_counter = buf[NREP * 2 * ch:NREP * 2 * ch + 1].view(torch.int32)
    return v


TAILS = {"enabled": os.environ.get("PCAA_BN_TAIL", "1") != "0", "taken": 0, "standalone": 0}


class BnTailFwd:
    def __init__(self, count, lin_bias, bn, ch, sync=None, update_running=True):
        self.count, self.lin_bias, self.bn, self.ch, self.sync, self.update_running = count, lin_bias, bn, ch, sync, update_running
        self.out = None
        self.armed = False
        self.count_out = count

    def arm(self, stats):
        counter = getattr(stats, "_pcaa_counter", None)
        if self.sync is not None or counter is None or not TAILS["enabled"]:
            return
        dev, bn, ch = stats.device, self.bn, self.ch
        scale = torch.empty(ch, dtype=torch.float32, device=dev)
        self.out = (scale, torch.empty_like(scale), torch.empty_like(scale), torch.empty_like(scale))
        rm = bn.running_mean if self.update_running else None
        rv = bn.running_var if self.update_running else None
        nbt = bn.num_batches_tracked if self.update_running else None
        check(_lib.load().pcaa_bn_tail_arm_fwd(_p(stats), NREP, int(self.count), _p(self.lin_bias), _p(bn.weight), _p(bn.bias),
                                               _p(rm), _p(rv), _p(nbt), BN_MOMENTUM if bn.momentum is None else bn.momentum,
                                               bn.eps, *(_p(t) for t in self.out), ch, _p(counter)), "pcaa_bn_tail_arm_fwd")
        self.armed = True

    def resolve(self, stats):
        lib = _lib.load()
        if self.armed and not lib.pcaa_bn_tail_pending():
            TAILS["taken"] += 1
            return self.out
        if self.armed:
            lib.pcaa_bn_tail_disarm()
        count = self.sync(stats, self.count) if self.sync is not None else self.count
        self.count_out = count
        TAILS["standalone"] += 1
        self.out = bn_finalize(stats, count, self.lin_bias, self.bn, self.ch, self.update_running)
        return self.out


class BnTailBwd:
    def __init__(self, count, bn, mean, rstd, ch, dgamma=None, dbeta=None, sync=None):
        self.count, self.bn, self.mean, self.rstd, self.ch, self.sync = count, bn, mean, rstd, ch, sync
        self.dgamma, self.dbeta = dgamma, dbeta
        self.out = None
        self.armed = False
# ... 450 lines not shown
    return max(1, min(s, K // (4 * bk) if K >= 4 * bk else 1))


def cast_bf16(W2d, want_plain=True, want_transposed=True, out=None):
    _chk(W2d, "cast_bf16.W", torch.float32, 2)
    R, C = W2d.shape
    if out is not None:
        _chk(out, "cast_bf16.out", torch.bfloat16, 2)
        if tuple(out.shape) != (R, C):
            raise ValueError("cast_bf16: out shape")
    w = out if out is not None else (torch.empty((R, C), dtype=torch.bfloat16, device=W2d.device) if want_plain else None)
    wt = torch.empty((C, R), dtype=torch.bfloat16, device=W2d.device) if want_transposed else None
    check(_lib.load().pcaa_cast_bf16(_p(W2d), _p(w), _p(wt), R, C, _s()), "pcaa_cast_bf16")
    return w, wt


def pointnet_in_ok(C, cout):
    return 1 <= C <= 8 and cout % 4 == 0 and cout <= 1024 and 256 % (cout // 4) == 0


def pointnet_in_fwd(x2d, W2d, bias, out_dtype, stats=None, tail=None):
    _chk(x2d, "pointnet_in.x", torch.float32, 2)
    _chk(W2d, "pointnet_in.W", torch.float32, 2)
    P, C = x2d.shape
    cout = W2d.shape[0]
    if W2d.shape[1] != C or not pointnet_in_ok(C, cout):
        raise ValueError(f"pointnet_in_fwd: unsupported shape C={C} cout={cout}")
    if out_dtype is None:
        if stats is None:
            raise ValueError("pointnet_in_fwd: statistics-only call needs stats")
        if tail is not None:
            tail.arm(stats)
        check(_lib.load().pcaa_pointnet_in_fwd(_p(x2d), C, _p(W2d), None, None, PCAA_F32, P, cout, _p(stats), NREP,
                                               _s()), "pcaa_pointnet_in_fwd(stats)")
        if tail is not None:
            tail.resolve(stats)
        return None
    y = torch.empty((P, cout), dtype=out_dtype, device=x2d.device)
    if tail is not None and stats is not None:
        tail.arm(stats)
    check(_lib.load().pcaa_pointnet_in_fwd(_p(x2d), C, _p(W2d), _p(bias), _p(y), _dt(y), P, cout, _p(stats), NREP, _s()),
          "pcaa_pointnet_in_fwd")
    if tail is not None and stats is not None:
        tail.resolve(stats)
    return y


def pointnet_in_apply(x2d, W2d, scale, shift, out_dtype):
    _chk(x2d, "pointnet_in_apply.x", torch.float32, 2)
    _chk(W2d, "pointnet_in_apply.W", torch.float32, 2)
    P, C = x2d.shape
    cout = W2d.shape[0]
    if W2d.shape[1] != C or not pointnet_in_ok(C, cout):
        raise ValueError(f"pointnet_in_apply: unsupported shape C={C} cout={cout}")
    if out_dtype == SplitImage.dtype:
        a = split_image_empty(P, cout, x2d.device, SPLIT_SCALE_ACT)
        check(_lib.load().pcaa_pointnet_in_apply(_p(x2d), C, _p(W2d), _p(scale), _p(shift), _p(a.img), PCAA_SPLIT_F16, P,
                                                 cout, _s()), "pcaa_pointnet_in_apply(split)")
        return a
    a = torch.empty((P, cout), dtype=out_dtype, device=x2d.device)
    check(_lib.load().pcaa_pointnet_in_apply(_p(x2d), C, _p(W2d), _p(scale), _p(shift), _p(a), _dt(a), P, cout, _s()),
          "pcaa_pointnet_in_apply")
    return a


def pointnet_in_bwd_stats(da, x2d, W2d, scale, shift, mean, rstd, tail=None):
    _chk(da, "pointnet_in_bwd_stats.da", dim=2)
    _chk(x2d, "pointnet_in_bwd_stats.x", torch.float32, 2)
    P, cout = da.shape
    C = x2d.shape[1]
    if x2d.shape[0] != P or tuple(W2d.shape) != (cout, C) or not pointnet_in_ok(C, cout):
        raise ValueError("pointnet_in_bwd_stats: unsupported shape")
    stats = new_stats(cout, da.device)
    if tail is not None:
        tail.arm(stats)
    check(_lib.load().pcaa_pointnet_in_bwd_stats(_p(da), _dt(da), _p(x2d), C, _p(W2d), _p(scale), _p(shift), _p(mean),
                                                 _p(rstd), _p(stats), NREP, P, cout, _s()),
          "pcaa_pointnet_in_bwd_stats")
    if tail is not None:
        tail.resolve(stats)
    return stats


def points_moments(x2d):
    _chk(x2d, "points_moments.x", torch.float32, 2)
    lib = _lib.load()
    n = lib.pcaa_points_moments_size()
    mom = STATS_POOL.take_raw(n) if (STATS_POOL is not None and STATS_POOL.buf.device == x2d.device) else None
    if mom is None:
        mom = torch.zeros(n, dtype=torch.float64, device=x2d.device)
    else:
        mom = mom[:n]
    check(lib.pcaa_points_moments(_p(x2d), x2d.shape[1], x2d.shape[0], _p(mom), _s()), "pcaa_points_moments")
    return mom


def pointnet_in_moment_coeffs(x2d, W2d, lin_bias, bn, mom=None, update_running=True):
    _chk(x2d, "pointnet_in_moment_coeffs.x", torch.float32, 2)
    P, C = x2d.shape
    cout = W2d.shape[0]
    if mom is None:
        mom = points_moments(x2d)
    tail = BnTailFwd(P, lin_bias, bn, cout, update_running=update_running)
    stats = mom
    stats._pcaa_counter = mom
    tail.arm(stats)
    if not tail.armed:
        raise RuntimeError("pointnet_in_moment_coeffs: the carried finalize is switched off")
    check(_lib.load().pcaa_pointnet_in_moment_stats(_p(mom), _p(W2d), C, cout, _s()), "pcaa_pointnet_in_moment_stats")
    TAILS["taken"] += 1
    return tail.out + (mom,)


def pointnet_in_bwd_onepass(da, x2d, W2d, scale, shift, mean, rstd, tail, mom=None, out=None):
    _chk(da, "pointnet_in_bwd_onepass.da", dim=2)
    _chk(x2d, "pointnet_in_bwd_onepass.x", torch.float32, 2)
    P, cout = da.shape
    C = x2d.shape[1]
    if x2d.shape[0] != P or tuple(W2d.shape) != (cout, C) or not pointnet_in_ok(C, cout):
        raise ValueError("pointnet_in_bwd_onepass: unsupported shape")
    lib = _lib.load()
    if mom is None:
        mom = points_moments(x2d)
    pivot_mom, pivot_count = mom, P
    if tail.sync is not None:
        pivot_mom = mom.clone()
        pivot_count = tail.sync(pivot_mom, P)
    stats = new_stats(cout, da.device)
    g_rows = lib.pcaa_pointnet_in_bwd_g_rows(P)
    G = torch.empty((g_rows, cout, C), dtype=torch.float32, device=da.device)
    tail.arm(stats)
    check(lib.pcaa_pointnet_in_bwd_onepass_rows(_p(da), _dt(da), _p(x2d), C, _p(W2d), _p(scale), _p(shift), _p(mean),
                                                _p(rstd), _p(stats), NREP, _p(G), P, cout, _p(pivot_mom), 1.0 / pivot_count,
                                                _s()), "pcaa_pointnet_in_bwd_onepass_rows")
    coef, _, _ = tail.resolve(stats)
    if out is None:
        out = torch.empty((cout, C), dtype=torch.float32, device=da.device)
    check(lib.pcaa_pointnet_in_bwd_combine(_p(G), g_rows, _p(W2d), _p(mom), _p(coef), _p(out), cout, C, P, _p(pivot_mom),
                                           1.0 / pivot_count, _s()), "pcaa_pointnet_in_bwd_combine")
    return out


def pointnet_in_bwd_wgrad(da, x2d, W2d, scale, shift, coef, out=None, out_is_zero=False, dz_is_pre=False):
    _chk(da, "pointnet_in_bwd_wgrad.da", dim=2)
    _chk(x2d, "pointnet_in_bwd_wgrad.x", torch.float32, 2)
    P, cout = da.shape
    C = x2d.shape[1]
    if x2d.shape[0] != P or tuple(W2d.shape) != (cout, C) or not pointnet_in_ok(C, cout):
        raise ValueError("pointnet_in_bwd_wgrad: unsupported shape")
    if out is None:
        out = torch.zeros((cout, C), dtype=torch.float32, device=da.device)
    elif not out_is_zero:
        out.zero_()
    check(_lib.load().pcaa_pointnet_in_bwd_wgrad(_p(da), _dt(da), _p(x2d), C, _p(W2d), _p(scale), _p(shift), _p(coef),
                                                 _p(out), P, cout, int(bool(dz_is_pre)), _s()),
          "pcaa_pointnet_in_bwd_wgrad")
    return out


def pointnet_in_wgrad(dy, x2d, out=None, out_is_zero=False):
    _chk(dy, "pointnet_in_wgrad.dy", dim=2)
    _chk(x2d, "pointnet_in_wgrad.x", torch.float32, 2)
    P, cout = dy.shape
    C = x2d.shape[1]
    if x2d.shape[0] != P or not pointnet_in_ok(C, cout):
        raise ValueError("pointnet_in_wgrad: unsupported shape")
    if out is None:
        out = torch.zeros((cout, C), dtype=torch.float32, device=dy.device)
    elif not out_is_zero:
        out.zero_()
    check(_lib.load().pcaa_pointnet_in_wgrad(_p(dy), _dt(dy), _p(x2d), C, _p(out), P, cout, _s()),
          "pcaa_pointnet_in_wgrad")
    return out


def bn_finalize(stats, count, lin_bias, bn, ch, update_running=True):
    dev = stats.device
    scale = torch.empty(ch, dtype=torch.float32, device=dev)
    shift = torch.empty_like(scale)
    mean = torch.empty_like(scale)
    rstd = torch.empty_like(scale)
    lib = _lib.load()
    rm = bn.running_mean if update_running else None
    rv = bn.running_var if update_running else None
    nbt = bn.num_batches_tracked if update_running else None
    check(lib.pcaa_bn_finalize(_p(stats), NREP, int(count), _p(lin_bias), _p(bn.weight), _p(bn.bias),
                               _p(rm), _p(rv), _p(nbt), BN_MOMENTUM if bn.momentum is None else bn.momentum,
                               bn.eps, _p(scale), _p(shift), _p(mean), _p(rstd), ch, _s()), "pcaa_bn_finalize")
    return scale, shift, mean, rstd


def bn_eval_coeffs(bn, ch, lin_bias=None):
# ... 496 lines not shown

def frames_from_raw(points, offsets, N, C, *, pick=None, seed=0, frame_key=None, standardize=True, divide_by_std=False,
                    n_out=None, pick_out=None, err_flag=None):
    if not isinstance(points, torch.Tensor) or points.dtype not in (torch.float32, torch.float64):
        raise TypeError("frames_from_raw.points: expected a float32 or float64 tensor")
    _chk(points, "frames_from_raw.points", None, 2)
    _chk(offsets, "frames_from_raw.offsets", torch.int32, 1)
    N, C, seed = int(N), int(C), int(seed)
    n = offsets.numel() - 1
    n_out = n if n_out is None else int(n_out)
    if points.shape[1] != 5 or n < 0 or n_out < n or not 1 <= N <= RAW_MAX_POINTS or not 1 <= C <= 5:
        raise ValueError(f"frames_from_raw: needs points [P, 5], offsets [n + 1], n_out >= n, 1 <= N <= {RAW_MAX_POINTS}, "
                         f"1 <= C <= 5; got points {tuple(points.shape)}, n={n}, n_out={n_out}, N={N}, C={C}")
    if not -2 ** 63 <= seed < 2 ** 63:
        raise ValueError("frames_from_raw: the seed must fit 64 bits")
    if pick is not None:
        _chk(pick, "frames_from_raw.pick", torch.int32, 2)
        if tuple(pick.shape) != (n, N):
            raise ValueError(f"frames_from_raw: pick must be [{n}, {N}], got {tuple(pick.shape)}")
    elif n:
        if frame_key is None:
            raise ValueError("frames_from_raw: without picks every frame needs its key (frame_key int32 [n, 2])")
        _chk(frame_key, "frames_from_raw.frame_key", torch.int32, 2)
        if tuple(frame_key.shape) != (n, 2):
            raise ValueError(f"frames_from_raw: frame_key must be [{n}, 2], got {tuple(frame_key.shape)}")
    if pick_out is not None:
        _chk(pick_out, "frames_from_raw.pick_out", torch.int32, 2)
        if tuple(pick_out.shape) != (n, N):
            raise ValueError(f"frames_from_raw: pick_out must be [{n}, {N}], got {tuple(pick_out.shape)}")
    if err_flag is not None:
        _chk(err_flag, "frames_from_raw.err_flag", torch.int32)
    out = torch.empty((n_out, N, C), dtype=torch.float32, device=points.device)
    if n_out:
        check(_lib.load().pcaa_frames_from_raw(
            _p(points), int(points.dtype == torch.float64), points.shape[0], _p(offsets), n, _p(pick),
            None if pick is not None else _p(frame_key), seed, N, C, int(bool(standardize)), int(bool(divide_by_std)),
            _p(out), n_out, _p(pick_out), _p(err_flag), _s()), "pcaa_frames_from_raw")
    return out


def stream_score(logits, sup_fv, means, run_start, win_stream, win_j, vote_pos, n_votes, threshold, k, n_labels,
                 n_classes, hist_lik, hist_pred):
    _chk(logits, "stream_score.logits", torch.float32, 2)
    _chk(sup_fv, "stream_score.sup_fv", torch.float32, 2)
    _chk(means, "stream_score.means", torch.float32, 2)
    _chk(hist_lik, "stream_score.hist_lik", torch.float64, 2)
    _chk(hist_pred, "stream_score.hist_pred", torch.int64, 2)
    for t, name in ((run_start, "run_start"), (win_stream, "win_stream"), (win_j, "win_j"), (vote_pos, "vote_pos")):
        _chk(t, "stream_score." + name, torch.int32, 1)
    nw, K = logits.shape
    D = sup_fv.shape[1]
    k, n_votes, n_runs = int(k), int(n_votes), run_start.numel() - 1
    if (sup_fv.shape[0] != nw or means.shape[1] != D or win_stream.numel() != nw or win_j.numel() != nw
            or vote_pos.numel() != nw or k < 1 or tuple(hist_lik.shape) != tuple(hist_pred.shape)
            or hist_lik.shape[1] != k or not 0 <= n_votes <= nw or not (1 <= n_runs <= nw or nw == 0)):
        raise ValueError("stream_score: shapes do not describe one tick")
    dev = logits.device
    preds = torch.empty(nw, dtype=torch.int64, device=dev)
    lik = torch.empty(nw, dtype=torch.float64, device=dev)
    votes = torch.empty(n_votes, dtype=torch.int64, device=dev)
    if nw:
        check(_lib.load().pcaa_stream_score(
            _p(logits), _p(sup_fv), _p(means), _p(run_start), n_runs, _p(win_stream), _p(win_j), _p(vote_pos), nw, K, D,
            means.shape[0], ctypes.c_double(float(threshold)), k, int(n_labels), int(n_classes), _p(hist_lik),
            _p(hist_pred), hist_lik.shape[0], _p(preds), _p(lik), _p(votes) if n_votes else None, n_votes, _s()),
            "pcaa_stream_score")
    return preds, lik, votes


def dtc_im2col(a, B, T, Cin, d):
    _chk(a, "im2col.a", torch.float32, 2)
    col = torch.empty((B * T, 3 * Cin), dtype=torch.float32, device=a.device)
    check(_lib.load().pcaa_dtc_im2col(_p(a), _p(col), B, T, Cin, d, _s()), "pcaa_dtc_im2col")
    return col


def dtc_col2im(dcol, B, T, Cin, d):
    _chk(dcol, "col2im.dcol", torch.float32, 2)
    da = torch.empty((B * T, Cin), dtype=torch.float32, device=dcol.device)
    check(_lib.load().pcaa_dtc_col2im(_p(dcol), _p(da), B, T, Cin, d, _s()), "pcaa_dtc_col2im")
    return da


def chamfer(preds, gts, want_grad, grad_scale=1.0, grad_per_b=None):
    for t, nm in ((preds, "preds"), (gts, "gts")):
        if not t.is_cuda or t.dtype != torch.float32 or t.dim() != 4:
            raise RuntimeError(f"chamfer: {nm} must be a 4-D float32 tensor on the HIP device")
    if preds.shape != gts.shape:
        raise ValueError("chamfer: shape mismatch")
    B, C, T, N = preds.shape
    fl = torch.empty((B, T), dtype=torch.float32, device=preds.device)
    dp = torch.empty((B, C, T, N), dtype=torch.float32, device=preds.device) if want_grad else None
    ds = dp.stride() if want_grad else (0, 0, 0, 0)
    ps, gs = preds.stride(), gts.stride()
    check(_lib.load().pcaa_chamfer_fwd_bwd(_p(preds), ps[0], ps[1], ps[2], ps[3], _p(gts), gs[0], gs[1], gs[2], gs[3],
                                           B, T, N, C, _p(fl), _p(dp), ds[0], ds[1], ds[2], ds[3],
                                           float(grad_scale), _p(grad_per_b), _s()), "pcaa_chamfer_fwd_bwd")
    return fl, dp


def cross_entropy(logits, target=None, want_loss=True, want_grad=False, grad_scale=1.0, want_preds=False,
                  err_flag=None):
    _chk(logits, "ce.logits", torch.float32, 2)
    B, K = logits.shape
    if target is not None:
        _chk(target, "ce.target", torch.int64, 1)
        if target.shape[0] != B:
            raise ValueError(f"cross_entropy: {target.shape[0]} targets for {B} rows of logits")
        if err_flag is None:
            lo, hi = int(target.min().item()), int(target.max().item())
            if lo < 0 or hi >= K:
                raise IndexError(f"cross_entropy: target {lo if lo < 0 else hi} is out of bounds for {K} classes")
        else:
            _chk(err_flag, "ce.err_flag", torch.int32)
    dev = logits.device
    loss = torch.empty((), dtype=torch.float32, device=dev) if (want_loss and target is not None) else None
    dl = torch.empty_like(logits) if want_grad else None
    pr = torch.empty(B, dtype=torch.int64, device=dev) if want_preds else None
    check(_lib.load().pcaa_cross_entropy(_p(logits), _p(target), B, K, _p(loss), _p(dl), float(grad_scale), _p(pr),
                                         _p(err_flag) if target is not None else None, _s()),
          "pcaa_cross_entropy")
    return loss, dl, pr


def orced_heads_fwd(x4, Wmu, bmu, Wlv, blv, eps, Wc, bc):
    for t, nm in ((x4, "x4"), (Wmu, "Wmu"), (Wlv, "Wlv"), (eps, "eps"), (Wc, "Wc")):
        _chk(t, f"orced_heads_fwd.{nm}", torch.float32, 2)
    B, d_in = x4.shape
    L, K = Wmu.shape[0], Wc.shape[0]
    lib = _lib.load()
    if (tuple(Wmu.shape) != (L, d_in) or tuple(Wlv.shape) != (L, d_in) or tuple(eps.shape) != (B, L)
            or tuple(Wc.shape) != (K, L) or not lib.pcaa_orced_heads_supported(B, K, d_in, L)):
        raise ValueError("orced_heads_fwd: unsupported shapes")
    mu = torch.empty((B, L), dtype=torch.float32, device=x4.device)
    logvar, sup = torch.empty_like(mu), torch.empty_like(mu)
    logits = torch.empty((B, K), dtype=torch.float32, device=x4.device)
    check(lib.pcaa_orced_heads_fwd(_p(x4), _p(Wmu), _p(bmu), _p(Wlv), _p(blv), _p(eps), _p(Wc), _p(bc), _p(mu), _p(logvar),
                                   _p(sup), _p(logits), B, K, d_in, L, _s()), "pcaa_orced_heads_fwd")
    return logits, sup, mu, logvar


def orced_heads_bwd(x4, eps, logvar, sup, Wmu, Wlv, Wc, d_logits, d_sup, d_mu, d_logvar, need_dx=True):
    B, d_in = x4.shape
    L, K = Wmu.shape[0], Wc.shape[0]
    dev = x4.device
    for t in (d_logits, d_sup, d_mu, d_logvar):
        if t is not None:
            _chk(t, "orced_heads_bwd.grad", torch.float32, 2)
    ws = torch.empty(2 * B * L, dtype=torch.float32, device=dev)
    dWmu, dWlv = torch.empty_like(Wmu), torch.empty_like(Wlv)
    dbmu = torch.empty(L, dtype=torch.float32, device=dev)
    dblv = torch.empty_like(dbmu)
    dWc = torch.empty_like(Wc)
    dbc = torch.empty(K, dtype=torch.float32, device=dev)
    dx4 = torch.empty_like(x4) if need_dx else None
    check(_lib.load().pcaa_orced_heads_bwd(_p(x4), _p(eps), _p(logvar), _p(sup), _p(Wmu), _p(Wlv), _p(Wc), _p(d_logits),
                                           _p(d_sup), _p(d_mu), _p(d_logvar), _p(ws), _p(dWmu), _p(dbmu), _p(dWlv), _p(dblv),
                                           _p(dWc), _p(dbc), _p(dx4), B, K, d_in, L, _s()), "pcaa_orced_heads_bwd")
    return dx4, dWmu, dbmu, dWlv, dblv, dWc, dbc


def orced_kl(mu, logvar, mu_k, want_loss=True, gscale=None):
    for t in (mu, logvar, mu_k):
        _chk(t, "orced_kl", torch.float32, 2)
    B, L = mu.shape
    if tuple(logvar.shape) != (B, L) or tuple(mu_k.shape) != (B, L):
        raise ValueError("orced_kl: shape mismatch")
    loss = torch.empty((), dtype=torch.float32, device=mu.device) if want_loss else None
    grads = (torch.empty_like(mu), torch.empty_like(mu), torch.empty_like(mu)) if gscale is not None else (None, None, None)
    check(_lib.load().pcaa_orced_kl(_p(mu), _p(logvar), _p(mu_k), _p(loss), _p(grads[0]), _p(grads[1]), _p(grads[2]),
                                    float(gscale if gscale is not None else 0.0), B, L, _s()), "pcaa_orced_kl")
    return loss, grads


def _disc_params(m):
    lin = (m.model[0], m.model[2], m.model[4])
    return [lin[0].weight, lin[0].bias, lin[1].weight, lin[1].bias, lin[2].weight, lin[2].bias]


def disc_workspace(B, K, device):
    n = _lib.load().pcaa_disc_workspace_bytes(B, K)
# ... 13 lines not shown


def disc_backward(x, label, params, gout, want_dx=True, want_dlabel=False, want_params=True, grads_out=None, dx_out=None):
    B, K = label.shape
    _chk(gout, "disc.gout", torch.float32)
    if gout.numel() != B:
        raise ValueError("disc_backward: gout size")
    dev = x.device
    if dx_out is not None:
        _chk(dx_out, "disc.dx_out", torch.float32)
        if tuple(dx_out.shape) != tuple(x.shape):
            raise ValueError("disc_backward: dx_out must have x's shape")
    dx = (dx_out if dx_out is not None else torch.empty_like(x)) if want_dx else None
    dl = torch.empty_like(label) if want_dlabel else None
    if want_params:
        grads = grads_out if grads_out is not None else [torch.empty_like(p) for p in params]
        ws = disc_workspace(B, K, dev)
    else:
        grads = [None] * 6
        ws = None
    check(_lib.load().pcaa_disc_backward(_p(x), _p(label), B, K, *[_p(p) for p in params], _p(gout), _p(dx), _p(dl),
                                         *[_p(g) for g in grads], _p(ws), 0 if ws is None else ws.numel() * 4, _s()),
          "pcaa_disc_backward")
    return dx, dl, (grads if want_params else None)


def disc_backward_backward(x, label, params, gout, gbar, want_dx=True, want_dlabel=False, want_dgout=True,
                           want_params=True):
    for t, nm in ((x, "x"), (label, "label"), (gout, "gout"), (gbar, "gbar")):
        _chk(t, f"disc_bb.{nm}", torch.float32)
    B, K = label.shape
    if x.shape != (B, 32) or gbar.shape != (B, 32) or gout.numel() != B:
        raise ValueError("disc_backward_backward: shapes")
    dev = x.device
    dx2 = torch.empty_like(x) if want_dx else None
    dl2 = torch.empty_like(label) if want_dlabel else None
    dgo = torch.empty(B, dtype=torch.float32, device=dev) if want_dgout else None
    grads = [torch.empty_like(p) for p in params] if want_params else [None] * 6
    ws = disc_workspace(B, K, dev)
    check(_lib.load().pcaa_disc_backward_backward(_p(x), _p(label), B, K, *[_p(p) for p in params], _p(gout), _p(gbar),
                                                  _p(dx2), _p(dl2), _p(dgo), *[_p(g) for g in grads], _p(ws),
                                                  ws.numel() * 4, _s()), "pcaa_disc_backward_backward")
    return dx2, dl2, dgo, (grads if want_params else None)


def disc_wgan_gp(z, fv, label, alphas, params, gp_weight, grads_out=None, want_dz=False, losses_out=None):
    for t, nm in ((z, "z"), (fv, "fv"), (label, "label"), (alphas, "alphas")):
        _chk(t, f"wgan.{nm}", torch.float32)
    B, K = label.shape
    if z.shape != (B, 32) or fv.shape != (B, 32) or alphas.numel() != B:
        raise ValueError("disc_wgan_gp: shapes")
    dev = z.device
    losses = torch.empty(2, dtype=torch.float32, device=dev) if losses_out is None else _chk(losses_out, "wgan.losses_out", torch.float32)
    if losses.numel() != 2:
        raise ValueError("disc_wgan_gp: losses_out must hold 2 floats")
    grads = grads_out if grads_out is not None else [torch.empty_like(p) for p in params]
    ws = disc_workspace(B, K, dev)
    dz = torch.empty_like(z) if want_dz else None
    check(_lib.load().pcaa_disc_wgan_gp(_p(z), _p(fv), _p(label), _p(alphas), B, K, *[_p(p) for p in params],
                                        float(gp_weight), _p(losses), *[_p(g) for g in grads], _p(dz), _p(ws),
                                        ws.numel() * 4, _s()), "pcaa_disc_wgan_gp")
    if want_dz:
        return losses, grads, dz
    return losses, grads


def adam_step_(p, g, m, v, lr, b1, b2, eps, step, grad_scale=1.0, max_blocks=0):
    for t, nm in ((p, "p"), (g, "g"), (m, "m"), (v, "v")):
        _chk(t, f"adam.{nm}", torch.float32)
    n = p.numel()
    if not (g.numel() == n and m.numel() == n and v.numel() == n):
        raise ValueError("adam_step_: size mismatch")
    check(_lib.load().pcaa_adam_step(_p(p), _p(g), _p(m), _p(v), n, float(lr), float(b1), float(b2), float(eps),
                                     int(step), float(grad_scale), int(max_blocks), _s()), "pcaa_adam_step")


def adam_advance_(step_dev, coef_dev, lr, b1, b2):
    _chk(step_dev, "adam.step_dev", torch.int32)
    _chk(coef_dev, "adam.coef_dev", torch.float32)
    if step_dev.numel() != 1 or coef_dev.numel() != 2:
        raise ValueError("adam_advance_: step_dev is int32[1], coef_dev float32[2]")
    check(_lib.load().pcaa_adam_advance(_p(step_dev), _p(coef_dev), float(lr), float(b1), float(b2), _s()),
          "pcaa_adam_advance")


def adam_step_dev_(p, g, m, v, b1, b2, eps, coef_dev, grad_scale=1.0, max_blocks=0):
    for nm, t in (("p", p), ("g", g), ("m", m), ("v", v)):
        _chk(t, f"adam.{nm}", torch.float32)
    _chk(coef_dev, "adam.coef_dev", torch.float32)
    n = p.numel()
    if not (g.numel() == m.numel() == v.numel() == n) or coef_dev.numel() != 2:
        raise ValueError("adam_step_dev_: size mismatch")
    check(_lib.load().pcaa_adam_step_dev(_p(p), _p(g), _p(m), _p(v), n, float(b1), float(b2), float(eps),
                                         _p(coef_dev), float(grad_scale), int(max_blocks), _s()),
          "pcaa_adam_step_dev")


def adam_step_dev_g16_(p, g16, m, v, b1, b2, eps, coef_dev, grad_scale=1.0, max_blocks=0):
    for nm, t in (("p", p), ("m", m), ("v", v)):
        _chk(t, f"adam_g16.{nm}", torch.float32)
    _chk(g16, "adam_g16.g", torch.bfloat16)
    _chk(coef_dev, "adam_g16.coef_dev", torch.float32)
    n = p.numel()
    if not (g16.numel() == m.numel() == v.numel() == n) or coef_dev.numel() != 2:
        raise ValueError("adam_step_dev_g16_: size mismatch")
    check(_lib.load().pcaa_adam_step_dev_g16(_p(p), _p(g16), _p(m), _p(v), n, float(b1), float(b2), float(eps),
                                             _p(coef_dev), float(grad_scale), int(max_blocks), _s()),
          "pcaa_adam_step_dev_g16")


def heads_supported(B, K, d_in, d_sup, d_head, d_proj, backward):
    return bool(_lib.load().pcaa_heads_supported(int(B), int(K), int(d_in), int(d_sup), int(d_head), int(d_proj),
                                                 1 if backward else 0))


def heads_fwd(x4, W1, b1, Wh, bh, W2, b2, Wg=None, bg=None):
    _chk(x4, "heads_fwd.x4", torch.float32, 2)
    for nm, t in (("W1", W1), ("b1", b1), ("W2", W2), ("b2", b2)):
        _chk(t, f"heads_fwd.{nm}", torch.float32)
    B, K = x4.shape[0], W2.shape[0]
    d_head = Wh.shape[0] if Wh is not None else 0
    d_proj = Wg.shape[0] if Wg is not None else 0
    if (tuple(W1.shape) != (32, x4.shape[1]) or W2.shape[1] != (d_head or 32)
            or not heads_supported(B, K, x4.shape[1], 32, d_head, d_proj, False)):
        raise ValueError(f"heads_fwd: unsupported shapes x4 {tuple(x4.shape)} W1 {tuple(W1.shape)} W2 {tuple(W2.shape)}")
    dev = x4.device
    sup = torch.empty((B, 32), dtype=torch.float32, device=dev)
    h = torch.empty((B, d_head), dtype=torch.float32, device=dev) if Wh is not None else None
    logits = torch.empty((B, K), dtype=torch.float32, device=dev)
    hproj = torch.empty((B, d_proj), dtype=torch.float32, device=dev) if Wg is not None else None
    check(_lib.load().pcaa_heads_fwd(_p(x4), _p(W1), _p(b1), _p(Wh), _p(bh), _p(W2), _p(b2), _p(Wg), _p(bg),
                                     _p(sup), _p(h), _p(logits), _p(hproj), B, K, _s()), "pcaa_heads_fwd")
    return sup, h, logits, hproj


def heads_bwd(x4, sup_fv, h, logits, hproj, W1, Wh, W2, Wg, d_logits, d_sup, d_hproj, outs=None):
    B, K = x4.shape[0], W2.shape[0]
    for nm, t in (("x4", x4), ("sup_fv", sup_fv), ("logits", logits), ("W1", W1), ("W2", W2)):
        _chk(t, f"heads_bwd.{nm}", torch.float32)
    for nm, t, shape in (("d_logits", d_logits, (B, K)), ("d_sup", d_sup, (B, 32)), ("d_hproj", d_hproj, (B, 64))):
        if t is not None:
            _chk(t, f"heads_bwd.{nm}", torch.float32)
            if tuple(t.shape) != shape:
                raise ValueError(f"heads_bwd.{nm}: shape {tuple(t.shape)}, expected {shape}")
    outs = dict(outs or {})
    dev = x4.device
    want = {"dW1": W1, "db1": W1.shape[0], "dW2": W2, "db2": K}
    if Wh is not None:
        want.update(dWh=Wh, dbh=Wh.shape[0])
    if d_hproj is not None:
        want.update(dWg=Wg, dbg=Wg.shape[0])
    for k, like in want.items():
        if outs.get(k) is None:
            outs[k] = (torch.empty_like(like) if isinstance(like, torch.Tensor)
                       else torch.empty(like, dtype=torch.float32, device=dev))
        _chk(outs[k], f"heads_bwd.{k}", torch.float32)
    dx4 = torch.empty_like(x4)
    check(_lib.load().pcaa_heads_bwd(_p(x4), _p(sup_fv), _p(h), _p(logits), _p(hproj), _p(W1), _p(Wh), _p(W2),
                                     _p(Wg), _p(d_logits), _p(d_sup), _p(d_hproj), _p(outs["dW1"]), _p(outs["db1"]),
                                     _p(outs.get("dWh")), _p(outs.get("dbh")), _p(outs["dW2"]), _p(outs["db2"]),
                                     _p(outs.get("dWg")), _p(outs.get("dbg")), _p(dx4), B, K, _s()), "pcaa_heads_bwd")
    return outs, dx4


def dtc_conv_supported(T, cin, cout):
    return bool(_lib.load().pcaa_dtc_conv_supported(int(T), int(cin), int(cout)))


def dtc_conv_fwd(src, scale, shift, W2d, B, T, dilation, stats=None, want_col=False, tail=None, bf16=False, win_row=None):
    _chk(src, "dtc_conv_fwd.src", torch.float32, 2)
    _chk(W2d, "dtc_conv_fwd.W", torch.float32, 2)
    rows, cin = src.shape
    cout = W2d.shape[0]
    if win_row is not None:
        if not isinstance(win_row, WindowRows):
            raise TypeError("dtc_conv_fwd: win_row must be an ops.WindowRows (it carries the host-side range check)")
        if stats is not None or want_col or tail is not None:
            raise ValueError("dtc_conv_fwd: a windowed source is eval-only (no statistics, no im2col)")
        if len(win_row) != B or win_row.T != T or win_row.table_rows != rows:
            raise ValueError(f"dtc_conv_fwd: win_row describes {len(win_row)} windows of {win_row.T} rows in a table of "
                             f"{win_row.table_rows}, got B={B} T={T} table {tuple(src.shape)}")
        rows = B * T
    if rows != B * T or W2d.shape[1] != cin * 3 or not dtc_conv_supported(T, cin, cout):
        raise ValueError(f"dtc_conv_fwd: unsupported shapes src {tuple(src.shape)} W {tuple(W2d.shape)} B={B} T={T}")
    if scale is not None:
        _chk(scale, "dtc_conv_fwd.scale", torch.float32)
        _chk(shift, "dtc_conv_fwd.shift", torch.float32)
        if scale.numel() != cin or shift.numel() != cin:
            raise ValueError("dtc_conv_fwd: scale/shift length")
    if stats is not None:
        _chk(stats, "dtc_conv_fwd.stats", torch.float64)
        if tuple(stats.shape) != (NREP, 2, cout):
            raise ValueError("dtc_conv_fwd: stats shape")
    y = torch.empty((rows, cout), dtype=torch.float32, device=src.device)
    col = torch.empty((rows, cin * 3), dtype=torch.float32, device=src.device) if want_col else None
    lib = _lib.load()
    ksplit = lib.pcaa_dtc_conv_ksplit(B, cin, cout)
    if ksplit > 1:
        stride = rows * cout
        dst = torch.empty(ksplit * stride, dtype=torch.float32, device=src.device)
        dst_stats, split = None, (ksplit, stride)
    else:
        dst, dst_stats, split = y, stats, (1, 0)
        if tail is not None and stats is not None:
            tail.arm(stats)
    operands = (_p(src), _p(scale), _p(shift), _p(W2d), _p(dst))
    shape = (B, T, cin, cout, int(dilation))
    if win_row is None:
        fwd = lib.pcaa_dtc_conv_fwd_bf16 if bf16 else lib.pcaa_dtc_conv_fwd
        rc = fwd(*operands, _p(col), _p(dst_stats), NREP, *shape, *split, _s())
    elif not win_row.segments:
        fwd = lib.pcaa_dtc_conv_fwd_win_bf16 if bf16 else lib.pcaa_dtc_conv_fwd_win
        rc = fwd(*operands, _p(col), _p(dst_stats), NREP, *shape, *split,
                 _p(win_row.dev), win_row.table_rows, win_row.ring_rows, _s())
    else:
        fwd = lib.pcaa_dtc_conv_fwd_seg_bf16 if bf16 else lib.pcaa_dtc_conv_fwd_seg
        rc = fwd(*operands, *shape, *split, _p(win_row.dev), win_row.segments, win_row.ring_rows, _s())
    check(rc, "pcaa_dtc_conv_fwd")
    if ksplit > 1 and stats is not None:
        check(lib.pcaa_splitk_reduce_stats(_p(dst), ksplit, stride, _p(y), _p(stats), NREP, rows, cout, _s()),
              "pcaa_splitk_reduce_stats")
    elif ksplit > 1:
        check(lib.pcaa_splitk_reduce(_p(dst), ksplit, stride, stride, _p(y), 0, _s()), "pcaa_splitk_reduce")
    if tail is not None and stats is not None:
        tail.resolve(stats)
    return y, col


def dtc_conv_dgrad(dy, W2d, B, T, cin, dilation, dz=None, y=None, coef=None, want_dy=False, below=None, tail=None,
                   bf16=False):
    _chk(W2d, "dtc_conv_dgrad.W", torch.float32, 2)
    cout = W2d.shape[0]
    rows = B * T
    src = dy if dy is not None else dz
    _chk(src, "dtc_conv_dgrad.dy/dz", torch.float32, 2)
    if tuple(src.shape) != (rows, cout) or tuple(W2d.shape) != (cout, cin * 3) or T > 32 or cin % 4 or cout % 4:
        raise ValueError(f"dtc_conv_dgrad: unsupported shapes {tuple(src.shape)} W {tuple(W2d.shape)} B={B} T={T}")
    if dy is None:
        _chk(y, "dtc_conv_dgrad.y", torch.float32, 2)
        _chk(coef, "dtc_conv_dgrad.coef", torch.float32, 2)
        if tuple(y.shape) != (rows, cout) or tuple(coef.shape) != (3, cout):
            raise ValueError("dtc_conv_dgrad: y / coef shapes")
    lib = _lib.load()
    dev = src.device
    out = torch.empty((rows, cin), dtype=torch.float32, device=dev)
    dy_out = torch.empty((rows, cout), dtype=torch.float32, device=dev) if (want_dy and dy is None) else None
    ks = lib.pcaa_dtc_conv_dgrad_ksplit(B, cin, cout)
    dgrad = lib.pcaa_dtc_conv_dgrad_bf16 if bf16 else lib.pcaa_dtc_conv_dgrad
    stats = None
    ep = [None] * 5
    if below is not None:
        if ks > 1:
            raise ValueError("dtc_conv_dgrad: the fused epilogue needs cout <= 512")
        for t in below:
            _chk(t, "dtc_conv_dgrad.below", torch.float32)
        if tuple(below[0].shape) != (rows, cin) or any(t.numel() != cin for t in below[1:]):
            raise ValueError("dtc_conv_dgrad: below shapes")
        ep = list(below)
        stats = new_stats(cin, dev)
    if ks > 1:
        stride = rows * cin
        slabs = torch.empty(ks * stride, dtype=torch.float32, device=dev)
        check(dgrad(_p(dy), _p(dz), _p(y), _p(coef), _p(dy_out), _p(W2d), _p(slabs), None, None, None,
                                      None, None, None, NREP, B, T, cin, cout, int(dilation), ks, stride, _s()),
              "pcaa_dtc_conv_dgrad")
        check(lib.pcaa_splitk_reduce(_p(slabs), ks, stride, stride, _p(out), 0, _s()), "pcaa_splitk_reduce")
    else:
        if tail is not None and stats is not None:
            tail.arm(stats)
        check(dgrad(_p(dy), _p(dz), _p(y), _p(coef), _p(dy_out), _p(W2d), _p(out), *[_p(t) for t in ep],
                                      _p(stats), NREP, B, T, cin, cout, int(dilation), 1, 0, _s()),
              "pcaa_dtc_conv_dgrad")
        if tail is not None and stats is not None:
            tail.resolve(stats)
    return out, stats, (dy if dy is not None else dy_out)
```

opensetgaitrecognition_pcaa_amd/train.py:

```python
import itertools
import math
import os
import pickle

import numpy as np
import torch

from . import constants
from . import dist as pdist
from . import functional as F_hip
from . import ops
from ._lib import ACT_ELU
from .models import CGDecoder, CGDiscriminator, CGEncoder, GaussianMeanLearner
from .utils import sample_distant_points, save_model

_ALIGN = 64


_SIDE_STREAMS = {}


_SIDE_ADAM_AT = os.environ.get("PCAA_SIDE_ADAM_AT", "dec_bwd")


def _side_streams(device):
    if device.type != "cuda":
        return None, None, None
    key = device.index if device.index is not None else torch.cuda.current_device()
    if key not in _SIDE_STREAMS:
        side, small = torch.cuda.Stream(device=device), torch.cuda.Stream(device=device)
        layout = os.environ.get("PCAA_STREAM_LAYOUT", "separate")
        if layout == "critic_on_wgrad":
            _SIDE_STREAMS[key] = (side, small, small)
        elif layout == "critic_on_side":
            _SIDE_STREAMS[key] = (side, side, small)
        else:
            _SIDE_STREAMS[key] = (side, small, torch.cuda.Stream(device=device))
    return _SIDE_STREAMS[key]


class StepCount:

    def __init__(self, device):
        self.step = 0
        self.step_dev = torch.zeros(1, dtype=torch.int32, device=device)
        self.coef_dev = torch.zeros(2, dtype=torch.float32, device=device)

    def advance(self, lr, b1, b2):
        self.step += 1
        ops.adam_advance_(self.step_dev, self.coef_dev, lr, b1, b2)

    def set(self, step):
        self.step = int(step)
        self.step_dev.fill_(self.step)


class _CompressedWork:

    def __init__(self, work, dst32, src16):
        self.work, self.dst32, self.src16, self.done = work, dst32, src16, False

    def wait(self, widen=True):
        self.work.wait()
        if not self.done and widen:
            self.dst32.copy_(self.src16)
            self.done = True


class FlatBuffer:

    def __init__(self, named_params, device, padded_shapes=None, tail_multiple=None):
        self.names, self.offsets, self.sizes, self.params = [], [], [], []
        padded_shapes = padded_shapes or {}
        total = 0
        for name, p in named_params:
            self.names.append(name)
            self.offsets.append(total)
            n = int(torch.Size(padded_shapes[name]).numel()) if name in padded_shapes else p.numel()
            self.sizes.append(n)
            self.params.append(p)
            total += (n + _ALIGN - 1) // _ALIGN * _ALIGN
        if tail_multiple is not None:
            start = self.offsets[self.names.index(tail_multiple[0])]
            total = start + (total - start + tail_multiple[1] - 1) // tail_multiple[1] * tail_multiple[1]
        self.total = total
        self.p = torch.zeros(total, dtype=torch.float32, device=device)
        self.g = torch.zeros(total, dtype=torch.float32, device=device)
        self.m = torch.zeros(total, dtype=torch.float32, device=device)
        self.v = torch.zeros(total, dtype=torch.float32, device=device)
        self.grad_views = {}
        self.padded = {}
        with torch.no_grad():
            for name, p, o, n in zip(self.names, self.params, self.offsets, self.sizes):
                if name in padded_shapes:
                    shp = tuple(padded_shapes[name])
                    full_p, full_g = self.p[o:o + n].view(shp), self.g[o:o + n].view(shp)
                    window = tuple(slice(0, d) for d in p.shape)
                    full_p[window].copy_(p.detach())
                    p.data = full_p[window]
                    self.grad_views[name] = full_g[window]
                    self.padded[name] = (full_p, full_g)
                    continue
                self.p[o:o + n].copy_(p.detach().reshape(-1))
                p.data = self.p[o:o + n].view(p.shape)
                self.grad_views[name] = self.g[o:o + n].view(p.shape)
# ... 147 lines not shown
        pads = {}
        if self.decoder is not None:
            r64 = lambda v: (v + 63) // 64 * 64
            lins = self.decoder.dense_layers()
            if any(l.weight.shape[0] % 64 for l in lins):
                for i, l in enumerate(lins, start=1):
                    n_out, n_in = l.weight.shape
                    kp = n_in if i == 1 else r64(n_in)
                    pads[f"G.dense{i}.weight"] = (r64(n_out), kp)
                    pads[f"G.dense{i}.bias"] = (r64(n_out),)
        self._zero = self._dp_zero_arg and self.pg is not None
        self._zero_chunks = 4
        tail = None
        if self.decoder is None:
            self._zero = False
        if self._zero:
            first_dec = next(n for n, _ in g_named if n.startswith("G."))
            tail = (first_dec, pdist.zero_tail_multiple(self.world, self._zero_chunks, _ALIGN))
        self.flat_g = FlatBuffer(g_named, self.device, padded_shapes=pads, tail_multiple=tail)
        if pads:
            from types import SimpleNamespace
            self.decoder._pcaa_pad = [
                SimpleNamespace(weight=self.flat_g.padded[f"G.dense{i}.weight"][0],
                                bias=self.flat_g.padded[f"G.dense{i}.bias"][0])
                for i in range(1, len(self.decoder.dense_layers()) + 1)]
        d_named = [("D." + n, p) for n, p in self.discriminator.named_parameters()]
        if self.learn_centroids:
            d_named = [("ML." + n, p) for n, p in self.mean_learner.named_parameters()] + d_named
        self.flat_d = FlatBuffer(d_named, self.device)
        if self.variant == "v1":
            self._zero_means = torch.zeros((self.K, self.L), dtype=torch.float32, device=self.device)
            ml = [i for i, nm in enumerate(self.flat_d.names) if nm.startswith("ML.")]
            self._ml_end = self.flat_d.offsets[len(ml)] if ml and len(ml) < len(self.flat_d.offsets) else 0
        self._d_params = ops._disc_params(self.discriminator)
        self._d_grads = [self.flat_d.grad_views["D." + n] for n, _ in self.discriminator.named_parameters()]
        self._dec_grads = {} if self.decoder is None else {
            n: (self.flat_g.padded["G." + n][1] if "G." + n in self.flat_g.padded else self.flat_g.grad_views["G." + n])
            for n, _ in self.decoder.named_parameters() if n.startswith("dense")}
        self._enc_grads = {n: self.flat_g.grad_views["E." + n] for n, _ in self.encoder.named_parameters()}
        n_enc = sum(1 for nm in self.flat_g.names if nm.startswith("E."))
        enc_end = self.flat_g.offsets[n_enc] if n_enc < len(self.flat_g.offsets) else self.flat_g.total
        self._enc_region = self.flat_g.g[:enc_end]
        sup_idx = [i for i, nm in enumerate(self.flat_g.names)
                   if nm.startswith("E.MLP_head.") or nm.startswith("E.MLP_sup2.")]
        assert sup_idx == list(range(sup_idx[0], sup_idx[-1] + 1)) and sup_idx[-1] == n_enc - 1
        self._sup_range = (self.flat_g.offsets[sup_idx[0]], enc_end)
        self._tail_region = self.flat_g.g[enc_end:]
        dec_names = [i for i, nm in enumerate(self.flat_g.names) if nm.startswith("G.")]
        self._dec_start = self.flat_g.offsets[dec_names[0]] if dec_names else self.flat_g.total
        self._dec_fused = {}
        if self.decoder is not None:
            fg = self.flat_g
            for i in range(2, len(self.decoder.dense_layers()) + 1):
                nm = f"G.dense{i}.weight"
                k = fg.names.index(nm)
                o, n = fg.offsets[k], fg.sizes[k]
                shp = tuple(fg.padded[nm][0].shape) if nm in fg.padded else tuple(fg.params[k].shape)
                self._dec_fused[i] = (o, (o + n + _ALIGN - 1) // _ALIGN * _ALIGN,
                                      fg.p[o:o + n].view(shp), fg.m[o:o + n].view(shp), fg.v[o:o + n].view(shp))
        self._dec_w16 = {}
        self.w16_casts = 0
        self._side_adam_blocks = 256
        self._dp_chunks = 4
        self._side, self._aux, self._wg = _side_streams(self.device)
        if self._zero:
            n = (self.flat_g.total - self._dec_start) // self._zero_chunks
            self._zero_len = n
            import torch.distributed as dist
            self._zero_slices = pdist.zero_slices(self._dec_start, self.flat_g.total, self.world, self._zero_chunks,
                                                  dist.get_rank(self.pg))
            self._zero_g = [torch.empty(n // self.world, dtype=torch.float32, device=self.device)
                            for _ in range(self._zero_chunks)]
            self._zero_p = [torch.empty(n // self.world, dtype=torch.float32, device=self.device)
                            for _ in range(self._zero_chunks)]
            if self.grad_compress == "bf16":
                self._zero_g16 = [torch.empty(n // self.world, dtype=torch.bfloat16, device=self.device)
                                  for _ in range(self._zero_chunks)]
        self._g16_direct = set()
        if self.grad_compress == "bf16" and self._xchg is not None:
            self._g16 = torch.zeros(self.flat_g.total, dtype=torch.bfloat16, device=self.device)
            self._dec_grads16 = {i: (lo, self._g16[lo:lo + Wv.numel()].view(Wv.shape))
                                 for i, (lo, hi, Wv, mv, vv) in self._dec_fused.items()}
        self._stats_pool = ops.StatsPool(self.device)
        self._flat_ready = True
        if self.pg is not None and self.world > 1:
            self.sync_replicas()

    @torch.no_grad()
    def sync_replicas(self, src_rank=0):
        import torch.distributed as dist
        if self.pg is None or self.world == 1:
            return
        src = dist.get_global_rank(self.pg, src_rank)
        flat = []
        for fb in (self.flat_g, self.flat_d):
            flat += [fb.p, fb.m, fb.v, fb.count.step_dev, fb.count.coef_dev, fb.sup_count.step_dev,
                     fb.sup_count.coef_dev]
        lo_hi = [(fb.p.data_ptr(), fb.p.data_ptr() + fb.p.numel() * 4) for fb in (self.flat_g, self.flat_d)]
        rest = []
        for mod in self.modules().values():
            for t in list(mod.parameters()) + list(mod.buffers()):
                if not any(lo <= t.data_ptr() < hi for lo, hi in lo_hi):
                    rest.append(t.data)
        if self.discriminator_means is not None:
            rest.append(self.discriminator_means)
        for t in flat + rest:
            dist.broadcast(t, src=src, group=self.pg)
        for fb in (self.flat_g, self.flat_d):
            for c in (fb.count, fb.sup_count):
                c.step = int(c.step_dev.item())

    def check(self):
        if int(self._err.item()):
            raise IndexError(f"PCAATrainer: a ground-truth label was outside [0, {self.K})")
        ops.range_check(self.device)

    def train(self):
        for m in self.modules().values():
            m.train()

    def eval(self):
        for m in self.modules().values():
            m.eval()

    def _count(self, nbytes, kind="allreduce"):
        self.comm["collectives"] += 1
        self.comm["payload_bytes"] += int(nbytes)
        self.comm[kind + "_bytes"] = self.comm.get(kind + "_bytes", 0) + int(nbytes)

    def _allreduce(self, t, async_op=False):
        if self._collective() and t.numel():
            in_dec = (t.data_ptr() >= self.flat_g.g.data_ptr() + 4 * self._dec_start
                      and t.data_ptr() < self.flat_g.g.data_ptr() + 4 * self.flat_g.total)
            off = (t.data_ptr() - self.flat_g.g.data_ptr()) // 4 if in_dec else -1
            if self.grad_compress == "bf16" and in_dec and (t.numel() >= self._COMPRESS_MIN or off in self._g16_direct):
                g16 = self._g16[off:off + t.numel()]
                if off not in self._g16_direct:
                    g16.copy_(t)
                self._count(2 * t.numel())
                work = self._xchg.all_reduce(g16, async_op=async_op)
                if not async_op:
                    t.copy_(g16)
                    return None
                return _CompressedWork(work, t, g16)
            assert off not in self._g16_direct, "a bf16-direct gradient bucket reached the fp32 all-reduce"
            self._count(t.numel() * t.element_size())
            return self._xchg.all_reduce(t, async_op=async_op)
        return None

    def _collective(self):
        return self._xchg is not None and (self.world > 1 or self._force_collectives)

    def _advance_g(self, supervise):
        b1, b2 = self.betas_g()
        self.flat_g.advance(self.cfg["LR"], b1, b2)
        if supervise:
            self.flat_g.sup_count.advance(self.cfg["LR"], b1, b2)
        else:
            self._sup_split = True

    def _adam_g(self, lo, hi, supervise, gs, max_blocks=0):
        b1, b2 = self.betas_g()
        lr, fg = self.cfg["LR"], self.flat_g
        a, b = max(lo, self._sup_range[0]), min(hi, self._sup_range[1])
        if a >= b or (supervise and not self._sup_split):
            fg.adam(lr, b1, b2, grad_scale=gs, lo=lo, hi=hi, advance=False, max_blocks=max_blocks)
            return
        fg.adam(lr, b1, b2, grad_scale=gs, lo=lo, hi=a, advance=False, max_blocks=max_blocks)
        if supervise:
            fg.adam(lr, b1, b2, grad_scale=gs, lo=a, hi=b, advance=False, count=fg.sup_count)
        fg.adam(lr, b1, b2, grad_scale=gs, lo=b, hi=hi, advance=False, max_blocks=max_blocks)

    def _w16_active(self, mode, B, collective):
        if (self.decoder is None or not self.fused_decoder_update or collective or self._side is None or mode != "bf16"
                or os.environ.get("PCAA_DEC_W16", "0") != "1"):
            return {}
        return {i: t for i, t in self._dec_fused.items() if F_hip._skinny(mode, B, t[2].shape[0], t[2].shape[1])}

    def _refresh_w16(self, mode, B, collective):
        images = {}
        if self.decoder is None:
            return images
        params = self.decoder.dense_layers()
        active = self._w16_active(mode, B, collective)
        for i, t in self._dec_fused.items():
            if i not in active:
                if i in self._dec_w16:
                    self._dec_w16[i][1] = None
                continue
            Wv = t[2]
            ent = self._dec_w16.get(i)
            if ent is None:
                ent = self._dec_w16[i] = [torch.empty(Wv.shape, dtype=torch.bfloat16, device=Wv.device), None]
            ver = (Wv._version, params[i - 1].weight._version)
            if ent[1] != ver:
                ops.cast_bf16(Wv, want_transposed=False, out=ent[0])
                ent[1] = ver
                self.w16_casts += 1
            images[i] = ent[0]
        return images

    def step(self, pcs, gt, z0, alphas, supervise=True):
        with self._sync_bn():
            try:
                return self._step(pcs, gt, z0, alphas, supervise)
            finally:
                F_hip._SYNC_BN["events"] = None
                if self._step_events:
                    self.comm_events.append(self._step_events)
                self._step_events = None

    def _step(self, pcs, gt, z0, alphas, supervise):
        if not self._flat_ready:
            self.finalize()
        if self.discriminator_means is None and self.variant != "v1":
            raise RuntimeError("prior means not set: call sample_prior_means() / set_prior_means()")
        cfg = self.cfg
        B = pcs.shape[0]
        mode = self.precision or F_hip.get_precision()
        enc, dec = self.encoder, self.decoder
        gs = 1.0 / self.world
        ops.set_stats_pool(self._stats_pool)
        self._stats_pool.begin()
        self._enc_region.zero_()
        self.comm = {"collectives": 0, "payload_bytes": 0}
        F_hip._SYNC_BN["collectives"] = F_hip._SYNC_BN["payload_bytes"] = 0
        step_events = self._step_events = [] if self.time_comm else None
        F_hip._SYNC_BN["events"] = step_events if self._sync_bn_group is not None else None

        logits, sup_fv, st = F_hip.encoder_forward(enc, pcs, True, mode, gph=self.decoder_projection_head)
        F_hip.mark("heads_fwd")
        sup_loss, dlogits, preds = ops.cross_entropy(logits, gt, want_loss=True, want_grad=supervise,
                                                     grad_scale=1.0, want_preds=True, err_flag=self._err)
        adv = float(cfg["ADV_WEIGHT"])

        def critic_branch(outs=(None, None, None)):
            if self.variant == "v1":
                _, oh = ops.prior_sample(z0, self._zero_means, gt, self.K)
                if self.learn_centroids:
                    for n, p in self.mean_learner.named_parameters():
                        p.grad = self.flat_d.grad_views["ML." + n]
                    self.flat_d.g[:self._ml_end].zero_()
                    mus = self.mean_learner(oh)
                    z = z0 + mus.detach()
                    dl, _, dz = ops.disc_wgan_gp(z, sup_fv, oh, alphas.reshape(-1).contiguous(), self._d_params,
                                                 cfg["GP_WEIGHT"], grads_out=self._d_grads, want_dz=True, losses_out=outs[0])
                    mus.backward(dz)
                else:
                    with torch.no_grad():
                        z = z0 + self.mean_learner(oh)
                    dl, _ = ops.disc_wgan_gp(z, sup_fv, oh, alphas.reshape(-1).contiguous(), self._d_params,
                                             cfg["GP_WEIGHT"], grads_out=self._d_grads, losses_out=outs[0])
            else:
                z, oh = ops.prior_sample(z0, self.discriminator_means, gt, self.K)
                dl, _ = ops.disc_wgan_gp(z, sup_fv, oh, alphas.reshape(-1).contiguous(), self._d_params,
                                         cfg["GP_WEIGHT"], grads_out=self._d_grads, losses_out=outs[0])
            self._allreduce(self.flat_d.g)
            self.flat_d.adam(cfg["LR"], cfg["B1"], cfg["B2"], grad_scale=gs)
            synth = ops.disc_forward(sup_fv, oh, self._d_params)
            lg = ops.total(synth, -adv / B, out=outs[1])
            gout = torch.full((B,), -adv / B, dtype=torch.float32, device=self.device)
            ds, _, _ = ops.disc_backward(sup_fv, oh, self._d_params, gout, want_dx=True, want_params=False, dx_out=outs[2])
            return dl, lg, ds

        joined = None
        if self._aux is not None:
            main = ops.current_stream()
            fork = torch.cuda.Event()
            fork.record(main)
            outs = (torch.empty(2, dtype=torch.float32, device=self.device), torch.empty((), dtype=torch.float32, device=self.device),
                    torch.empty_like(sup_fv))
            for t in outs:
                t.record_stream(self._aux)
            with ops.on_stream(self._aux):
                self._aux.wait_event(fork)
                d_losses, loss_g, dsup = critic_branch(outs)
                joined = torch.cuda.Event()
                joined.record(self._aux)
        else:
            d_losses, loss_g, dsup = critic_branch()

        if self.variant == "v3":
            if joined is not None:
                ops.current_stream().wait_event(joined)
            F_hip.set_wgrad_stream(self._wg)
            try:
                F_hip.encoder_backward(enc, st, dlogits if supervise else None, dsup, gout=self._enc_grads)
            finally:
                F_hip.set_wgrad_stream(None)
            if self._wg is not None:
                ops.current_stream().wait_stream(self._wg)
            self._allreduce(self.flat_g.g)
            self._advance_g(supervise)
            self._adam_g(0, self.flat_g.total, supervise, gs)
            tot = loss_g + (sup_loss if supervise else 0.0)
            return {"d_loss": d_losses[0], "gp": d_losses[1], "rec_loss": None, "loss_g": loss_g,
                    "sup_loss": sup_loss, "tot_loss": tot, "preds": preds, "out_labels": logits, "sup_fvs": sup_fv}

        hproj = st.hproj if self.decoder_projection_head is not None else sup_fv
        w16 = self._refresh_w16(mode, B, self._collective())
        rec, acts = F_hip.decoder_forward(dec, hproj, mode, images=w16)
        F_hip.mark("dec_fwd")
        rec4 = rec.view(B, self.C, self.T, self.N)
        inv_bt = 1.0 / (B * self.T)
        frame_loss, drec = ops.chamfer(rec4, pcs, want_grad=True, grad_scale=inv_bt)
        rec_loss = ops.total(frame_loss, inv_bt)

        F_hip.mark("chamfer")
        F_hip.set_wgrad_stream(self._wg)
        if joined is not None and self.decoder_projection_head is None:
            ops.current_stream().wait_event(joined)
            joined = None
        dh = None
        collective = self._collective()
        early_buckets = []
        layer_hook = None
        zero = self._zero and collective and self._side is not None
        if zero:
            pass
        elif collective and self._wg is not None:
            fg = self.flat_g

            def layer_hook(layer):
                if layer < 2:
                    return
                lo = fg.offsets[fg.names.index(f"G.dense{layer}.weight")]
                nxt = f"G.dense{layer + 1}.weight"
                hi = fg.offsets[fg.names.index(nxt)] if nxt in fg.names else fg.total
                self._wg.wait_stream(ops.current_stream())
                with ops.on_stream(self._wg):
                    early_buckets.append((lo, hi, self._allreduce(fg.g[lo:hi], async_op=True)))

        updates, fused_ranges, deferred = None, [], []
        exact_dec = mode in ("fp32", "fp16x3")
        if (self.fused_decoder_update and not collective and self._side is not None
                and (mode == "bf16" or (self.fused_exact and exact_dec))):
            for layer, (lo, hi, Wv, mv, vv) in self._dec_fused.items():
                if F_hip._skinny(mode, B, Wv.shape[0], Wv.shape[1]) or F_hip._skinny_exact(mode, B, Wv.shape[0], Wv.shape[1]):
                    updates = updates or {}
                    updates[layer] = lambda dz2, x, t=(Wv, mv, vv, w16.get(layer)): deferred.append((dz2, x) + t + (None,))
                    fused_ranges.append((lo, hi))
        gather = (collective and self._dp_gather and not zero and mode == "bf16" and self.fused_decoder_update
                  and self._side is not None and self.world <= ops.PACK_MAX_CHUNKS and B <= ops.PACK_ROWS)
        self.dp_scheme = "zero" if zero else ("gather" if gather else ("allreduce" if collective else "none"))
        if gather:
            def gather_update(layer, Wv, mv, vv):
                def cb(dz2, x):
                    key = (layer, self.world)
                    if key not in self._gather_bufs:
                        ce = ops.packed_chunk_elems(Wv.shape[0], Wv.shape[1])
                        self._gather_bufs[key] = (torch.zeros((self.world, ce), dtype=torch.bfloat16, device=self.device),
                                                  torch.empty(ce, dtype=torch.bfloat16, device=self.device))
                    packed_all, own = self._gather_bufs[key]
                    dzc, xc = (dz2 if dz2.stride(1) == 1 else dz2.contiguous()), (x if x.stride(1) == 1 else x.contiguous())
                    self._count(2 * packed_all.numel(), "gather")

                    def send():
                        ops.pack_rows_t16(dzc, xc, out=own)
                        return self._xchg.all_gather_into_tensor(packed_all.view(-1), own, async_op=True, tag=layer)
                    if self._wg is not None:
                        self._wg.wait_stream(ops.current_stream())
                        with ops.on_stream(self._wg):
                            dzc.record_stream(self._wg)
                            xc.record_stream(self._wg)
                            work = send()
                    else:
                        work = send()
                    deferred.append((packed_all, None, Wv, mv, vv, None, [work]))
                return cb

            for layer, (lo, hi, Wv, mv, vv) in self._dec_fused.items():
                if F_hip._skinny(mode, B, Wv.shape[0], Wv.shape[1]):
                    updates = updates or {}
                    updates[layer] = gather_update(layer, Wv, mv, vv)
                    fused_ranges.append((lo, hi))
            if layer_hook is not None:
                plain_hook, taken = layer_hook, set(updates or {})

                def layer_hook(layer):
                    if layer not in taken:
                        plain_hook(layer)
        if not set(w16) <= set(updates or {}):
            raise RuntimeError("PCAATrainer: a bf16 weight image is in use for a layer whose update is not fused")
        dec_grads = self._dec_grads
        self._g16_direct = set()
        if collective and layer_hook is not None and self.grad_compress == "bf16" and mode == "bf16":
            dec_grads = dict(dec_grads)
            for layer, (lo, view16) in self._dec_grads16.items():
                if updates and layer in updates:
# ... 104 lines not shown
                                                      exact=exact_dec)
                        if w16 is not None:
                            ops.cast_bf16(Wv, want_transposed=False, out=w16)
                    for lo, hi, work in pending:
                        if hi <= self._dec_start:
                            continue
                        g16 = None
                        if isinstance(work, _CompressedWork) and (lo % 4 == 0):
                            work.wait(widen=False)
                            work.done = True
                            g16 = self._g16
                        elif work is not None:
                            work.wait()
                        a = max(lo, self._dec_start)
                        for flo, fhi in sorted(fused_ranges) + [(hi, hi)]:
                            if flo > a:
                                self.flat_g.adam(cfg["LR"], cfg["B1"], cfg["B2"], grad_scale=gs, lo=a, hi=min(flo, hi),
                                                 advance=False, max_blocks=self._side_adam_blocks, g16=g16)
                            a = max(a, fhi)
                            if a >= hi:
                                break
                    ev = torch.cuda.Event()
                    ev.record(self._side)
                    done.append(ev)

            at = _SIDE_ADAM_AT
            if at == "pointnet":
                hook = launch_side_adam
            elif at == "heads":
                hook_heads = launch_side_adam
            else:
                launch_side_adam()
        try:
            gv = self.flat_g.grad_views
            F_hip.encoder_backward(enc, st, dlogits if supervise else None, dsup, gout=self._enc_grads,
                                   before_pointnet=hook, after_heads=hook_heads,
                                   gph=self.decoder_projection_head, d_hproj=dh,
                                   gph_gout=(gv["GPH.0.weight"], gv["GPH.0.bias"]) if dh is not None else None)
        finally:
            F_hip.set_wgrad_stream(None)
        if self._wg is not None:
            ops.current_stream().wait_stream(self._wg)
        ev_c0 = None
        if self.time_comm and collective:
            ev_c0 = torch.cuda.Event(enable_timing=True)
            ev_c0.record()
        self._allreduce(self.flat_g.g[:self._dec_start])
        for _, _, work in pending:
            if work is not None:
                work.wait()
        if ev_c0 is not None:
            ev_c1 = torch.cuda.Event(enable_timing=True)
            ev_c1.record()
            step_events.append((ev_c0, ev_c1))
        if zero:
            self._adam_g(0, self._dec_start, supervise, gs)
            if ev_c0 is not None:
                ev_g0 = torch.cuda.Event(enable_timing=True)
                ev_g0.record()
            for work in zero_gather:
                work.wait()
            if ev_c0 is not None:
                ev_g1 = torch.cuda.Event(enable_timing=True)
                ev_g1.record()
                step_events.append((ev_g0, ev_g1))
        elif early:
            self._adam_g(0, self._dec_start, supervise, gs)
            ev_j0 = None
            if ev_c0 is not None:
                ev_j0 = torch.cuda.Event(enable_timing=True)
                ev_j0.record()
            ops.current_stream().wait_event(done[0])
            if ev_j0 is not None:
                ev_j1 = torch.cuda.Event(enable_timing=True)
                ev_j1.record()
                step_events.append((ev_j0, ev_j1))
        else:
            self._advance_g(supervise)
            self._adam_g(0, self.flat_g.total, supervise, gs)

        F_hip.mark("adam+join")
        self.comm["collectives"] += F_hip._SYNC_BN.get("collectives", 0)
        self.comm["payload_bytes"] += F_hip._SYNC_BN.get("payload_bytes", 0)
        tot = rec_loss + loss_g + (sup_loss if supervise else 0.0)
        return {"d_loss": d_losses[0], "gp": d_losses[1], "rec_loss": rec_loss, "loss_g": loss_g,
                "sup_loss": sup_loss, "tot_loss": tot, "preds": preds, "out_labels": logits, "sup_fvs": sup_fv}

    def exposed_comm_us(self):
        return [sum(e0.elapsed_time(e1) for e0, e1 in pairs) * 1e3 for pairs in self.comm_events]

    def prefers_graph(self, B, N):
        return (self.can_graph() and (self._xchg is None or self._xchg.emulated or os.environ.get("PCAA_GRAPH") == "on")
                and B * self.T * N <= 80_000 and os.environ.get("PCAA_GRAPH", "auto") != "off")

    def can_graph(self):
        return (self.variant in ("v4", "base", "v3") and self.device.type == "cuda"
                and (self._xchg is None or self._xchg.capturable) and not self.time_comm)

    def step_graphed(self, pcs, gt, z0, alphas, supervise=True, warmup=2):
        if not self.can_graph():
            raise RuntimeError("PCAATrainer.step_graphed: this trainer's step cannot be captured (variant 1's autograd, a gloo "
                               "process group, or time_comm's timing events): use step()")
        if not supervise and not self._sup_split:
            self._sup_split = True
            self._graphs.clear()
        key = (tuple(pcs.shape), tuple(pcs.stride()), bool(supervise))
        ent = self._graphs.setdefault(key, {"eager": 0, "graph": None})
        if ent["graph"] is None:
            if ent["eager"] < warmup:
                ent["eager"] += 1
                return self.step(pcs, gt, z0, alphas, supervise)
            static = [torch.empty_like(pcs), torch.empty_like(gt), torch.empty_like(z0), torch.empty_like(alphas)]
            for dst, src in zip(static, (pcs, gt, z0, alphas)):
                dst.copy_(src)
            steps0 = (self.flat_g.step, self.flat_d.step)
            self._refresh_w16(self.precision or F_hip.get_precision(), pcs.shape[0], False)
            graph = torch.cuda.CUDAGraph()
            torch.cuda.synchronize(self.device)
            with torch.cuda.graph(graph, capture_error_mode="thread_local"):
                out = self.step(*static, supervise)
            assert (self.flat_g.step, self.flat_d.step) == (steps0[0] + 1, steps0[1] + 1)
            ent.update(graph=graph, static=static, out=out)
            graph.replay()
            return out
        for dst, src in zip(ent["static"], (pcs, gt, z0, alphas)):
            if dst.data_ptr() != src.data_ptr():
                dst.copy_(src, non_blocking=True)
        self._refresh_w16(self.precision or F_hip.get_precision(), pcs.shape[0], False)
        self.flat_g.step += 1
        self.flat_d.step += 1
        if supervise:
            self.flat_g.sup_count.step += 1
        ent["graph"].replay()
        return ent["out"]

    @torch.no_grad()
    def evaluate_batch(self, pcs, gt):
        mode = self.precision or F_hip.get_precision()
        logits, sup_fv, _ = F_hip.encoder_forward(self.encoder, pcs, False, mode)
        if self.decoder is None:
            ce, _, preds = ops.cross_entropy(logits, gt, want_loss=True, want_preds=True, err_flag=self._err)
            return None, ce, preds, sup_fv
        hproj = sup_fv
        if self.decoder_projection_head is not None:
            hproj = F_hip.linear_act_forward(sup_fv, self.decoder_projection_head[0], ACT_ELU)
        rec, _ = F_hip.decoder_forward(self.decoder, hproj, mode)
        B = pcs.shape[0]
        fl, _ = ops.chamfer(rec.view(B, self.C, self.T, self.N), pcs, want_grad=False)
        rec_loss = ops.total(fl, 1.0 / (B * self.T))
        ce, _, preds = ops.cross_entropy(logits, gt, want_loss=True, want_preds=True, err_flag=self._err)
        return rec_loss, ce, preds, sup_fv

    def save_checkpoints(self, folder, model_name, write=True):
        suffix = {"E": "_E", "G": "_G", "D": "_D", "GPH": "_GPH", "DPH": "_DPH", "ML": "_ML"}
        if write:
            for key, mod in self.modules().items():
                save_model(mod, os.path.join(folder, f"{model_name}{suffix[key]}.pt"))
        if self.mean_learner is not None:
            with self._sync_bn():
                cent = self.learned_centroids()
            if write:
                torch.save(cent, os.path.join(folder, "discriminator_means.pt"))
        elif self.variant == "v3" and write:
            torch.save(self.discriminator_means, os.path.join(folder, "discriminator_means.pt"))

    @torch.no_grad()
    def learned_centroids(self):
        return self.mean_learner(torch.eye(self.K, dtype=torch.float32, device=self.device))


class _NullRun:
    def finish(self):
        pass


def _wandb():
    try:
        import wandb
        return wandb
    except Exception:
        return None


class _EpochDraws:

    def __init__(self, L, device, process_group=None, rank=0, world=1):
        self.L, self.dev, self.pg, self.rank, self.world = int(L), device, process_group, rank, world
        self._z_host = self._a_host = None
        self._copied = None

    def draw(self, steps, gb):
        if steps <= 0:
            return None, None
        if self._z_host is None or self._z_host.shape[0] < steps or self._z_host.shape[1] != gb:
            pin = self.dev.type == "cuda"
            self._z_host = torch.empty((steps, gb, self.L), dtype=torch.float32, pin_memory=pin)
            self._a_host = torch.empty((steps, gb, 1), dtype=torch.float32, pin_memory=pin)
        elif self._copied is not None:
            self._copied.synchronize()
        z_np = self._z_host.numpy()
        for i in range(steps):
            z_np[i] = np.random.normal(0.0, 1.0, (gb, self.L))
            torch.rand(size=(gb, 1), out=self._a_host[i])
        z = self._z_host[:steps].to(self.dev, non_blocking=True)
        a = self._a_host[:steps].to(self.dev, non_blocking=True)
        if self.dev.type == "cuda":
            self._copied = torch.cuda.Event()
            self._copied.record()
        if self.world > 1:
            import torch.distributed as dist
            src = dist.get_global_rank(self.pg, 0)
            dist.broadcast(z, src=src, group=self.pg)
            dist.broadcast(a, src=src, group=self.pg)
            per = gb // self.world
            z = z[:, self.rank * per:(self.rank + 1) * per]
            a = a[:, self.rank * per:(self.rank + 1) * per]
        return z, a


def _run_loop(config, variant, dataset_factory=None, log_fn=None, process_group=None, sync_bn=False, device="cuda",
              timing=None):
    import time
    from .datasets import MSRadarDataset
    from .constants import SPLIT

    nmax_points = config["NMAX"]
    os.makedirs(f"models/{config['MODEL_NAME']}", exist_ok=True)
    if process_group is None or torch.distributed.get_rank(process_group) == 0:
        with open(os.path.join("models", config["MODEL_NAME"], "config.pkl"), "wb") as f:
            pickle.dump(config, f)

    rank, world = 0, 1
# ... 183 lines not shown
```

Before: 12330 sequences/s.

## Fuse step-begin zeroing with Adam advance, fast chamfer with fused total, cache gout

Replaces the stats-pool and encoder-region zeroing plus the Adam step-count advances with one step_begin kernel. Adds a fast LDS-resident Chamfer kernel that uses norm-expanded distances and a bitmask inverse nearest-neighbour scatter, with a last-block tail that reduces frame losses into the scalar total. Also caches the discriminator gout tensor, sums the losses in a tiny kernel, and adds a BN-stats tail to the split-K reduce. The intent is to cut kernel launches and host overhead in a launch-bound train step, at the cost of atomic-counter tail logic and more fp32 reassociation in Chamfer.

```diff
diff --git a/include/pcaa_hip.h b/include/pcaa_hip.h
--- a/include/pcaa_hip.h
+++ b/include/pcaa_hip.h
@@ -7,7 +7,7 @@
 extern "C" {
 #endif
 
-#define PCAA_ABI_VERSION 20
+#define PCAA_ABI_VERSION 21
 
 #define PCAA_OK 0
 #define PCAA_ERR_INVALID_ARG 1
@@ -91,6 +91,9 @@
                                  float* dW, int cout, int C, long P, const double* pivot_mom, double pivot_inv_count,
                                  void* stream);
 int pcaa_pointnet_in_moment_stats(const double* mom, const float* W, int C, int cout, void* stream);
+long pcaa_points_moments_rows_size(long P);
+int pcaa_points_moments_stats(const float* x, int C, long P, double* mom, double* rows, unsigned* counter,
+                              const float* W, int cout, void* stream);
 int pcaa_pointnet_in_bwd_wgrad(const void* da, int dtype, const float* x, int C, const float* W,
                                const float* scale, const float* shift, const float* coef, float* dW,
                                long P, int cout, int dz_is_pre ,
@@ -159,6 +162,12 @@
                          int B, int T, int N, int C, float* frame_loss,
                          float* dpreds, long d_sb, long d_sc, long d_st, long d_sn,
                          float grad_scale, const float* grad_per_b, void* stream);
+int pcaa_chamfer_fwd_bwd_total(const float* preds, long p_sb, long p_sc, long p_st, long p_sn,
+                               const float* gts, long g_sb, long g_sc, long g_st, long g_sn,
+                               int B, int T, int N, int C, float* frame_loss,
+                               float* dpreds, long d_sb, long d_sc, long d_st, long d_sn,
+                               float grad_scale, const float* grad_per_b, float total_scale, float* total_out,
+                               unsigned* counter, int variant, void* stream);
 int pcaa_cross_entropy(const float* logits, const long long* target, int B, int K,
                        float* loss, float* dlogits, float grad_scale, long long* preds,
                        int* err_flag, void* stream);
@@ -329,6 +338,9 @@
                    float lr, float beta1, float beta2, float eps, int step, float grad_scale,
                    int max_blocks, void* stream);
 int pcaa_adam_advance(int* step_dev, float* coef_dev, float lr, float beta1, float beta2, void* stream);
+int pcaa_step_begin(void* zero0, long bytes0, void* zero1, long bytes1, int* step_a, float* coef_a, int* step_b,
+                    float* coef_b, float lr, float beta1, float beta2, void* stream);
+int pcaa_sum3(const float* a, const float* b, const float* c, float* out, void* stream);
 int pcaa_adam_step_dev(float* param, const float* grad, float* exp_avg, float* exp_avg_sq, long n,
                        float beta1, float beta2, float eps, const float* coef_dev, float grad_scale,
                        int max_blocks, void* stream);
diff --git a/opensetgaitrecognition_pcaa_amd/csrc/elementwise.hip b/opensetgaitrecognition_pcaa_amd/csrc/elementwise.hip
--- a/opensetgaitrecognition_pcaa_amd/csrc/elementwise.hip
+++ b/opensetgaitrecognition_pcaa_amd/csrc/elementwise.hip
@@ -561,13 +561,39 @@
   }
 }
 
-__global__ void adam_coef_kernel(int* __restrict__ step, float* __restrict__ coef, float lr, float b1, float b2) {
+__device__ __forceinline__ void adam_coef_advance(int* step, float* coef, float lr, float b1, float b2) {
   const int t = *step + 1;
   *step = t;
   const double bc1 = 1.0 - pow((double)b1, (double)t);
   const double bc2 = 1.0 - pow((double)b2, (double)t);
   coef[0] = (float)((double)lr / bc1);
   coef[1] = (float)(1.0 / sqrt(bc2));
+}
+
+__global__ void adam_coef_kernel(int* __restrict__ step, float* __restrict__ coef, float lr, float b1, float b2) {
+  adam_coef_advance(step, coef, lr, b1, b2);
+}
+
+__global__ __launch_bounds__(256) void step_begin_kernel(uint4* __restrict__ z0, long q0, int r0, uint4* __restrict__ z1,
+                                                         long q1, int r1, int* step_a, float* coef_a, int* step_b,
+                                                         float* coef_b, float lr, float b1, float b2) {
+  const long stride = (long)gridDim.x * 256;
+  const long i = (long)blockIdx.x * 256 + threadIdx.x;
+  const uint4 z = {0u, 0u, 0u, 0u};
+  for (long k = i; k < q0; k += stride) z0[k] = z;
+  for (long k = i; k < q1; k += stride) z1[k] = z;
+  if (blockIdx.x != 0) return;
+  if ((int)threadIdx.x < r0) reinterpret_cast<unsigned*>(z0 + q0)[threadIdx.x] = 0u;
+  if ((int)threadIdx.x < r1) reinterpret_cast<unsigned*>(z1 + q1)[threadIdx.x] = 0u;
+  if (threadIdx.x == 0 && step_a) adam_coef_advance(step_a, coef_a, lr, b1, b2);
+  if (threadIdx.x == 1 && step_b) adam_coef_advance(step_b, coef_b, lr, b1, b2);
+}
+
+__global__ void sum3_kernel(const float* __restrict__ a, const float* __restrict__ b, const float* __restrict__ c,
+                            float* __restrict__ out) {
+  float t = a[0] + b[0];
+  if (c) t = t + c[0];
+  out[0] = t;
 }
 
 inline int grid_for(long work_items, int per_block = 256, int cap = 256 * 8) {
@@ -1037,8 +1063,9 @@
 __global__ __launch_bounds__(256) void splitk_reduce_stats_kernel(const float* __restrict__ slabs, int nsplit,
                                                                   long stride, float* __restrict__ out,
                                                                   double* __restrict__ stats, int nrep,
-                                                                  long rows, int ch) {
+                                                                  long rows, int ch, BnTail tail) {
   __shared__ f32x4 red[2][256];
+  __shared__ int tail_flag;
   const int qpr = ch >> 2, rl = 256 / qpr;
   const int cq = threadIdx.x % qpr, rlane = threadIdx.x / qpr;
   const int c = cq * 4;
@@ -1061,6 +1088,7 @@
     for (int l = 0; l < rl; ++l) v += (double)red[stat][l * qpr + (cc >> 2)][cc & 3];
     unsafeAtomicAdd(&stats[((long)(blockIdx.x % nrep) * 2 + stat) * ch + cc], v);
   }
+  bn_tail_run(tail, threadIdx.x, 256, gridDim.x, &tail_flag);
 }
 }
 
@@ -1069,7 +1097,7 @@
   PCAA_CHECK_ARG(slabs && out && stats && nsplit >= 1 && nrep >= 1 && rows >= 1, "pcaa_splitk_reduce_stats: bad args");
   PCAA_CHECK_ARG(ch_ok(ch) && (slab_stride % 4) == 0, "pcaa_splitk_reduce_stats: ch/4 must divide 256 (ch=%d)", ch);
   hipLaunchKernelGGL(splitk_reduce_stats_kernel, dim3((unsigned)cdiv(rows, 32)), dim3(256), 0, as_stream(stream),
-                     slabs, nsplit, slab_stride, out, stats, nrep, rows, ch);
+                     slabs, nsplit, slab_stride, out, stats, nrep, rows, ch, pcaa_take_bn_tail(stats));
   PCAA_RETURN_LAUNCH_STATUS("pcaa_splitk_reduce_stats");
 }
 
@@ -1133,6 +1161,29 @@
   PCAA_RETURN_LAUNCH_STATUS("pcaa_adam_advance");
 }
 
+extern "C" int pcaa_step_begin(void* zero0, long bytes0, void* zero1, long bytes1, int* step_a, float* coef_a,
+                               int* step_b, float* coef_b, float lr, float beta1, float beta2, void* stream) {
+  PCAA_CHECK_ARG(bytes0 >= 0 && bytes1 >= 0 && bytes0 % 4 == 0 && bytes1 % 4 == 0 && (zero0 || bytes0 == 0) &&
+                     (zero1 || bytes1 == 0),
+                 "pcaa_step_begin: regions are whole 32-bit words (%ld, %ld bytes)", bytes0, bytes1);
+  PCAA_CHECK_ARG(reinterpret_cast<uintptr_t>(zero0) % 16 == 0 && reinterpret_cast<uintptr_t>(zero1) % 16 == 0,
+                 "pcaa_step_begin: regions must start 16-byte aligned");
+  PCAA_CHECK_ARG((step_a == nullptr) == (coef_a == nullptr) && (step_b == nullptr) == (coef_b == nullptr),
+                 "pcaa_step_begin: a step count comes with its coefficients");
+  const long q0 = bytes0 / 16, q1 = bytes1 / 16;
+  const int grid = grid_for((q0 > q1 ? q0 : q1), 256, 256 * 8);
+  hipLaunchKernelGGL(step_begin_kernel, dim3(grid), dim3(256), 0, as_stream(stream), static_cast<uint4*>(zero0), q0,
+                     (int)(bytes0 % 16 / 4), static_cast<uint4*>(zero1), q1, (int)(bytes1 % 16 / 4), step_a, coef_a,
+                     step_b, coef_b, lr, beta1, beta2);
+  PCAA_RETURN_LAUNCH_STATUS("pcaa_step_begin");
+}
+
+extern "C" int pcaa_sum3(const float* a, const float* b, const float* c, float* out, void* stream) {
+  PCAA_CHECK_ARG(a && b && out, "pcaa_sum3: null pointer");
+  hipLaunchKernelGGL(sum3_kernel, dim3(1), dim3(1), 0, as_stream(stream), a, b, c, out);
+  PCAA_RETURN_LAUNCH_STATUS("pcaa_sum3");
+}
+
 extern "C" int pcaa_adam_step_dev(float* param, const float* grad, float* exp_avg, float* exp_avg_sq, long n,
                                   float beta1, float beta2, float eps, const float* coef_dev, float grad_scale,
                                   int max_blocks, void* stream) {
diff --git a/opensetgaitrecognition_pcaa_amd/csrc/losses.hip b/opensetgaitrecognition_pcaa_amd/csrc/losses.hip
--- a/opensetgaitrecognition_pcaa_amd/csrc/losses.hip
+++ b/opensetgaitrecognition_pcaa_amd/csrc/losses.hip
@@ -85,6 +85,171 @@
         if (nn[N + i] == n) g += 2.f * w * (pv - sg[i * MAXC + c]);
       db[c * d_sc + n * d_sn] = g;
     }
+  }
+}
+
+typedef float f32x2 __attribute__((ext_vector_type(2)));
+
+constexpr int CF_HEAD = 160;
+
+__host__ __device__ inline size_t chamfer_fast_lds(int N, bool grad) {
+  return CF_HEAD + (size_t)12 * N * sizeof(float) + (grad ? (size_t)N * (N / 32) * sizeof(unsigned) : 0);
+}
+
+template <int V>
+__global__ __launch_bounds__(CH_THREADS) void chamfer_fast_kernel(
+    const float* __restrict__ preds, long p_sb, long p_sc, long p_st,
+    const float* __restrict__ gts, long g_sb, long g_sc, long g_st,
+    int T, int N, int C, float* frame_loss,
+    float* __restrict__ dpreds, long d_sb, long d_sc, long d_st,
+    float grad_scale, const float* __restrict__ grad_per_b,
+    float* total_out, float total_scale, unsigned* counter) {
+  extern __shared__ __attribute__((aligned(16))) char smraw[];
+  double* dred = reinterpret_cast<double*>(smraw);
+  float* red = reinterpret_cast<float*>(smraw + 128);
+  int* flag = reinterpret_cast<int*>(smraw + 144);
+  float* sg = reinterpret_cast<float*>(smraw + CF_HEAD);
+  float* sp = sg + 4 * N;
+  float* rg = sp + 4 * N;
+  float* rp = rg + N;
+  int* nn = reinterpret_cast<int*>(rp + N);
+  unsigned* inv = reinterpret_cast<unsigned*>(nn + 2 * N);
+
+  const int tid = threadIdx.x;
+  const int frame = blockIdx.x;
+  const int b = frame / T, t = frame - b * T;
+  const float* pb = preds + b * p_sb + t * p_st;
+  const float* gb = gts + b * g_sb + t * g_st;
+
+  for (int c = 0; c < 4; ++c)
+    for (int n = tid; n < N; n += CH_THREADS) {
+      sg[c * N + n] = (c < C) ? gb[c * g_sc + n] : 0.f;
+      sp[c * N + n] = (c < C) ? pb[c * p_sc + n] : 0.f;
+    }
+  if (dpreds)
+    for (int e = tid; e < N * (N / 32); e += CH_THREADS) inv[e] = 0u;
+  __syncthreads();
+  for (int n = tid; n < N; n += CH_THREADS) {
+    float a = 0.f, q = 0.f;
+#pragma unroll
+    for (int c = 0; c < 4; ++c) {
+      a = fmaf(sg[c * N + n], sg[c * N + n], a);
+      q = fmaf(sp[c * N + n], sp[c * N + n], q);
+    }
+    rg[n] = a;
+    rp[n] = q;
+  }
+  __syncthreads();
+
+  const float w = grad_scale * (grad_per_b ? grad_per_b[b] : 1.f);
+  float loss = 0.f;
+  for (int item = tid; item < 2 * N; item += CH_THREADS) {
+    const bool dir1 = item < N;
+    const int me = dir1 ? item : item - N;
+    const float* mine = dir1 ? sp : sg;
+    const float* other = dir1 ? sg : sp;
+    const float* rother = dir1 ? rg : rp;
+    const float v0 = mine[me], v1 = mine[N + me], v2 = mine[2 * N + me], v3 = mine[3 * N + me];
+    const float rme = dir1 ? rp[me] : rg[me];
+    float best = 3.4e38f;
+    int bi = 0;
+    for (int o = 0; o < N; o += 4) {
+      const f32x4 x = *reinterpret_cast<const f32x4*>(other + o);
+      const f32x4 y = *reinterpret_cast<const f32x4*>(other + N + o);
+      const f32x4 z = *reinterpret_cast<const f32x4*>(other + 2 * N + o);
+      const f32x4 u = *reinterpret_cast<const f32x4*>(other + 3 * N + o);
+      const f32x4 r = *reinterpret_cast<const f32x4*>(rother + o);
+      float P[4];
+      if constexpr (V == 1) {
+#pragma unroll
+        for (int h = 0; h < 2; ++h) {
+          const f32x2 xx = h ? x.zw : x.xy, yy = h ? y.zw : y.xy, zz = h ? z.zw : z.xy, uu = h ? u.zw : u.xy;
+          const f32x2 rr = h ? r.zw : r.xy;
+          f32x2 dot = {0.f, 0.f};
+          dot = __builtin_elementwise_fma(xx, (f32x2){v0, v0}, dot);
+          dot = __builtin_elementwise_fma(yy, (f32x2){v1, v1}, dot);
+          dot = __builtin_elementwise_fma(zz, (f32x2){v2, v2}, dot);
+          dot = __builtin_elementwise_fma(uu, (f32x2){v3, v3}, dot);
+          const f32x2 pp = (rr + (f32x2){rme, rme}) - 2.f * dot;
+          P[2 * h] = pp.x;
+          P[2 * h + 1] = pp.y;
+        }
+      } else {
+#pragma unroll
+        for (int k = 0; k < 4; ++k) {
+          float dot = 0.f;
+          dot = fmaf(x[k], v0, dot);
+          dot = fmaf(y[k], v1, dot);
+          dot = fmaf(z[k], v2, dot);
+          dot = fmaf(u[k], v3, dot);
+          P[k] = (r[k] + rme) - 2.f * dot;
+        }
+      }
+#pragma unroll
+      for (int k = 0; k < 4; ++k)
+        if (P[k] < best) { best = P[k]; bi = o + k; }
+    }
+    loss += best;
+    nn[item] = bi;
+    if (dpreds && !dir1) atomicOr(&inv[(me >> 5) * N + bi], 1u << (me & 31));
+  }
+  loss = wave_sum(loss);
+  if ((tid & 63) == 0) red[tid >> 6] = loss;
+  __syncthreads();
+  if (tid == 0) {
+    float tot = 0.f;
+    for (int i = 0; i < CH_THREADS / 64; ++i) tot += red[i];
+    __hip_atomic_store(frame_loss + frame, tot, __ATOMIC_RELAXED, __HIP_MEMORY_SCOPE_AGENT);
+  }
+  if (dpreds) {
+    float* db = dpreds + b * d_sb + t * d_st;
+    for (int n = tid; n < N; n += CH_THREADS) {
+      float pv[4], g[4];
+      const int j = nn[n];
+#pragma unroll
+      for (int c = 0; c < 4; ++c) {
+        pv[c] = sp[c * N + n];
+        g[c] = 2.f * w * (pv[c] - sg[c * N + j]);
+      }
+      for (int k = 0; k < N / 32; ++k) {
+        unsigned m = inv[k * N + n];
+        while (m) {
+          const int i = k * 32 + __builtin_ctz(m);
+          m &= m - 1;
+#pragma unroll
+          for (int c = 0; c < 4; ++c) g[c] += 2.f * w * (pv[c] - sg[c * N + i]);
+        }
+      }
+#pragma unroll
+      for (int c = 0; c < 4; ++c)
+        if (c < C) db[c * d_sc + n] = g[c];
+    }
+  }
+  if (counter == nullptr) return;
+  asm volatile("s_waitcnt vmcnt(0)" ::: "memory");
+  __syncthreads();
+  if (tid == 0) {
+    const unsigned prev = __hip_atomic_fetch_add(counter, 1u, __ATOMIC_RELAXED, __HIP_MEMORY_SCOPE_AGENT);
+    *flag = prev == gridDim.x - 1 ? 1 : 0;
+  }
+  __syncthreads();
+  if (*flag == 0) return;
+  __builtin_amdgcn_fence(__ATOMIC_ACQUIRE, "wavefront");
+  if (tid == 0) __hip_atomic_store(counter, 0u, __ATOMIC_RELAXED, __HIP_MEMORY_SCOPE_AGENT);
+  const long nfr = gridDim.x;
+#pragma unroll
+  for (int k = 0; k < 1024 / CH_THREADS; ++k) {
+    double acc = 0.0;
+    for (long i = tid + k * CH_THREADS; i < nfr; i += 1024)
+      acc += (double)__hip_atomic_load(frame_loss + i, __ATOMIC_RELAXED, __HIP_MEMORY_SCOPE_AGENT);
+    acc = wave_sum_d(acc);
+    if ((tid & 63) == 0) dred[(tid >> 6) + k * (CH_THREADS / 64)] = acc;
+  }
+  __syncthreads();
+  if (tid == 0) {
+    double tt = 0.0;
+    for (int i = 0; i < 16; ++i) tt += dred[i];
+    total_out[0] = (float)(tt * (double)total_scale);
   }
 }
 
@@ -124,13 +289,29 @@
 
 }
 
-extern "C" int pcaa_chamfer_fwd_bwd(const float* preds, long p_sb, long p_sc, long p_st, long p_sn,
-                                    const float* gts, long g_sb, long g_sc, long g_st, long g_sn,
-                                    int B, int T, int N, int C, float* frame_loss, float* dpreds,
-                                    long d_sb, long d_sc, long d_st, long d_sn, float grad_scale,
-                                    const float* grad_per_b, void* stream) {
+extern "C" int pcaa_chamfer_fwd_bwd_total(const float* preds, long p_sb, long p_sc, long p_st, long p_sn,
+                                          const float* gts, long g_sb, long g_sc, long g_st, long g_sn,
+                                          int B, int T, int N, int C, float* frame_loss, float* dpreds,
+                                          long d_sb, long d_sc, long d_st, long d_sn, float grad_scale,
+                                          const float* grad_per_b, float total_scale, float* total_out,
+                                          unsigned* counter, int variant, void* stream) {
   PCAA_CHECK_ARG(preds && gts && frame_loss, "pcaa_chamfer_fwd_bwd: null pointer");
   PCAA_CHECK_ARG(B >= 1 && T >= 1 && N >= 1 && C >= 1 && C <= MAXC, "pcaa_chamfer_fwd_bwd: need 1<=C<=%d (C=%d)", MAXC, C);
+  PCAA_CHECK_ARG(variant >= 0 && variant <= 2, "pcaa_chamfer_fwd_bwd_total: variant must be 0, 1 or 2 (%d)", variant);
+  const bool fast = variant != 0 && C <= 4 && N % 64 == 0 && p_sn == 1 && g_sn == 1 && (!dpreds || d_sn == 1) &&
+                    chamfer_fast_lds(N, dpreds != nullptr) <= 64 * 1024;
+  if (fast) {
+    const bool tail = total_out != nullptr && counter != nullptr;
+    auto kern = variant == 1 ? chamfer_fast_kernel<1> : chamfer_fast_kernel<2>;
+    hipLaunchKernelGGL(kern, dim3((unsigned)(B * T)), dim3(CH_THREADS), chamfer_fast_lds(N, dpreds != nullptr),
+                       as_stream(stream), preds, p_sb, p_sc, p_st, gts, g_sb, g_sc, g_st, T, N, C, frame_loss, dpreds,
+                       d_sb, d_sc, d_st, grad_scale, grad_per_b, tail ? total_out : nullptr, total_scale,
+                       tail ? counter : nullptr);
+    hipError_t e = hipGetLastError();
+    if (e != hipSuccess) { pcaa_set_error("pcaa_chamfer_fwd_bwd: launch failed: %s", hipGetErrorString(e)); return PCAA_ERR_LAUNCH; }
+    if (tail || total_out == nullptr) return PCAA_OK;
+    return pcaa_sum(frame_loss, (long)B * T, total_scale, total_out, stream);
+  }
   const size_t lds = ((size_t)2 * N * MAXC + 4 * (size_t)N) * sizeof(float);
   PCAA_CHECK_ARG(lds <= 150 * 1024, "pcaa_chamfer_fwd_bwd: N=%d too large for one LDS tile", N);
   if (lds > 64 * 1024) {
@@ -141,7 +322,20 @@
   hipLaunchKernelGGL(chamfer_kernel, dim3((unsigned)(B * T)), dim3(CH_THREADS), lds, as_stream(stream),
                      preds, p_sb, p_sc, p_st, p_sn, gts, g_sb, g_sc, g_st, g_sn, T, N, C, frame_loss,
                      dpreds, d_sb, d_sc, d_st, d_sn, grad_scale, grad_per_b);
-  PCAA_RETURN_LAUNCH_STATUS("pcaa_chamfer_fwd_bwd");
+  hipError_t e = hipGetLastError();
+  if (e != hipSuccess) { pcaa_set_error("pcaa_chamfer_fwd_bwd: launch failed: %s", hipGetErrorString(e)); return PCAA_ERR_LAUNCH; }
+  if (total_out == nullptr) return PCAA_OK;
+  return pcaa_sum(frame_loss, (long)B * T, total_scale, total_out, stream);
+}
+
+extern "C" int pcaa_chamfer_fwd_bwd(const float* preds, long p_sb, long p_sc, long p_st, long p_sn,
+                                    const float* gts, long g_sb, long g_sc, long g_st, long g_sn,
+                                    int B, int T, int N, int C, float* frame_loss, float* dpreds,
+                                    long d_sb, long d_sc, long d_st, long d_sn, float grad_scale,
+                                    const float* grad_per_b, void* stream) {
+  return pcaa_chamfer_fwd_bwd_total(preds, p_sb, p_sc, p_st, p_sn, gts, g_sb, g_sc, g_st, g_sn, B, T, N, C, frame_loss,
+                                    dpreds, d_sb, d_sc, d_st, d_sn, grad_scale, grad_per_b, 0.f, nullptr, nullptr, 1,
+                                    stream);
 }
 
 extern "C" int pcaa_cross_entropy(const float* logits, const long long* target, int B, int K, float* loss,
diff --git a/opensetgaitrecognition_pcaa_amd/csrc/pointnet_in.hip b/opensetgaitrecognition_pcaa_amd/csrc/pointnet_in.hip
--- a/opensetgaitrecognition_pcaa_amd/csrc/pointnet_in.hip
+++ b/opensetgaitrecognition_pcaa_amd/csrc/pointnet_in.hip
@@ -375,6 +375,99 @@
   bn_tail_channel(t, o, s1, s2);
 }
 
+constexpr int MOM_ROW = 48;
+
+template <int CP>
+__global__ __launch_bounds__(256) void points_moments_rows_kernel(const float* __restrict__ x, int C, long P,
+                                                                  double* mom, double* rows, unsigned* counter,
+                                                                  const float* __restrict__ W, BnTail t) {
+  constexpr int NV = CP * (CP + 1) / 2 + CP;
+  __shared__ double red[4][NV];
+  __shared__ double moms[MAXC * MAXC + MAXC];
+  __shared__ int flag;
+  double a[NV];
+#pragma unroll
+  for (int i = 0; i < NV; ++i) a[i] = 0.0;
+  for (long r = (long)blockIdx.x * 256 + threadIdx.x; r < P; r += (long)gridDim.x * 256) {
+    double xv[CP];
+    if (CP == 4 && C == 4) {
+      const f32x4 v = load4(x + r * 4);
+      xv[0] = v.x; xv[1] = v.y; xv[2] = v.z; xv[3] = v.w;
+    } else {
+#pragma unroll
+      for (int c = 0; c < CP; ++c) xv[c] = c < C ? (double)x[r * C + c] : 0.0;
+    }
+    int i = 0;
+#pragma unroll
+    for (int k = 0; k < CP; ++k)
+#pragma unroll
+      for (int c = k; c < CP; ++c) { a[i] = fma(xv[k], xv[c], a[i]); ++i; }
+#pragma unroll
+    for (int c = 0; c < CP; ++c) a[i + c] += xv[c];
+  }
+#pragma unroll
+  for (int i = 0; i < NV; ++i) {
+    const double v = wave_sum_d(a[i]);
+    if ((threadIdx.x & 63) == 0) red[threadIdx.x >> 6][i] = v;
+  }
+  __syncthreads();
+  if (threadIdx.x < NV) {
+    const double v = red[0][threadIdx.x] + red[1][threadIdx.x] + red[2][threadIdx.x] + red[3][threadIdx.x];
+    __hip_atomic_store(rows + (long)blockIdx.x * MOM_ROW + threadIdx.x, v, __ATOMIC_RELAXED, __HIP_MEMORY_SCOPE_AGENT);
+  }
+  asm volatile("s_waitcnt vmcnt(0)" ::: "memory");
+  __syncthreads();
+  if (threadIdx.x == 0) {
+    const unsigned prev = __hip_atomic_fetch_add(counter, 1u, __ATOMIC_RELAXED, __HIP_MEMORY_SCOPE_AGENT);
+    flag = prev == gridDim.x - 1 ? 1 : 0;
+  }
+  __syncthreads();
+  if (flag == 0) return;
+  __builtin_amdgcn_fence(__ATOMIC_ACQUIRE, "wavefront");
+  if (threadIdx.x == 0) __hip_atomic_store(counter, 0u, __ATOMIC_RELAXED, __HIP_MEMORY_SCOPE_AGENT);
+  if (threadIdx.x < MAXC * MAXC + MAXC) moms[threadIdx.x] = 0.0;
+  __syncthreads();
+  if (threadIdx.x < NV) {
+    double v = 0.0;
+    const int nb = (int)gridDim.x;
+    int b = 0;
+    for (; b + 8 <= nb; b += 8) {
+      double u[8];
+#pragma unroll
+      for (int j = 0; j < 8; ++j) u[j] = bn_tail_ld(rows + (long)(b + j) * MOM_ROW + threadIdx.x);
+#pragma unroll
+      for (int j = 0; j < 8; ++j) v += u[j];
+    }
+    for (; b < nb; ++b) v += bn_tail_ld(rows + (long)b * MOM_ROW + threadIdx.x);
+    int i = threadIdx.x;
+    if (i < CP * (CP + 1) / 2) {
+      int k = 0;
+      while (i >= CP - k) { i -= CP - k; ++k; }
+      const int c = k + i;
+      moms[k * MAXC + c] = v;
+      if (c != k) moms[c * MAXC + k] = v;
+    } else {
+      moms[MAXC * MAXC + (i - CP * (CP + 1) / 2)] = v;
+    }
+  }
+  __syncthreads();
+  if (threadIdx.x < MAXC * MAXC + MAXC) mom[threadIdx.x] = moms[threadIdx.x];
+  if (t.kind != 1) return;
+  if (threadIdx.x == 0 && t.nbt != nullptr) *t.nbt += 1;
+  for (int o = threadIdx.x; o < t.ch; o += 256) {
+    double w[MAXC];
+    for (int k = 0; k < MAXC; ++k) w[k] = k < C ? (double)W[o * C + k] : 0.0;
+    double s1 = 0.0, s2 = 0.0;
+    for (int k = 0; k < C; ++k) {
+      s1 += w[k] * moms[MAXC * MAXC + k];
+      double row = 0.0;
+      for (int c = 0; c < C; ++c) row += moms[k * MAXC + c] * w[c];
+      s2 += w[k] * row;
+    }
+    bn_tail_channel(t, o, s1, s2);
+  }
+}
+
 __global__ __launch_bounds__(256) void pointnet_in_bwd_combine_kernel(const float* __restrict__ G, int g_rows,
                                                                       const float* __restrict__ W,
                                                                       const double* __restrict__ mom,
@@ -628,6 +721,30 @@
   PCAA_RETURN_LAUNCH_STATUS("pcaa_points_moments");
 }
 
+static long moments_grid(long P) {
+  long g = cdiv(P, 256 * 4);
+  return g > 512 ? 512 : g;
+}
+
+extern "C" long pcaa_points_moments_rows_size(long P) { return P >= 1 ? moments_grid(P) * MOM_ROW : 0; }
+
+extern "C" int pcaa_points_moments_stats(const float* x, int C, long P, double* mom, double* rows, unsigned* counter,
+                                         const float* W, int cout, void* stream) {
+  PCAA_CHECK_ARG(x && mom && rows && counter && C >= 1 && C <= MAXC && P >= 1, "pcaa_points_moments_stats: bad args");
+  BnTail t = {};
+  if (W != nullptr) {
+    t = pcaa_take_bn_tail(mom);
+    PCAA_CHECK_ARG(t.kind == 1 && t.ch == cout && cout >= 1, "pcaa_points_moments_stats: arm the forward finalize on `mom` "
+                   "first (pcaa_bn_tail_arm_fwd)");
+  }
+  const long g = moments_grid(P);
+  if (C <= 4) hipLaunchKernelGGL(points_moments_rows_kernel<4>, dim3((unsigned)g), dim3(256), 0, as_stream(stream), x, C, P,
+                                 mom, rows, counter, W, t);
+  else hipLaunchKernelGGL(points_moments_rows_kernel<8>, dim3((unsigned)g), dim3(256), 0, as_stream(stream), x, C, P, mom,
+                          rows, counter, W, t);
+  PCAA_RETURN_LAUNCH_STATUS("pcaa_points_moments_stats");
+}
+
 extern "C" int pcaa_pointnet_in_moment_stats(const double* mom, const float* W, int C, int cout, void* stream) {
   PCAA_CHECK_ARG(mom && W && C >= 1 && C <= MAXC && cout >= 1, "pcaa_pointnet_in_moment_stats: bad args");
   const BnTail t = pcaa_take_bn_tail(mom);
diff --git a/opensetgaitrecognition_pcaa_amd/ops.py b/opensetgaitrecognition_pcaa_amd/ops.py
--- a/opensetgaitrecognition_pcaa_amd/ops.py
+++ b/opensetgaitrecognition_pcaa_amd/ops.py
@@ -176,10 +176,12 @@
         self.buf = torch.zeros(capacity_doubles, dtype=torch.float64, device=device)
         self.off = 0
 
-    def begin(self):
-        if self.off:
-            self.buf[:self.off].zero_()
+    def begin(self, zero=True):
+        used = self.buf[:self.off]
+        if self.off and zero:
+            used.zero_()
         self.off = 0
+        return used
 
     def take_raw(self, n):
         n = (n + 1) // 2 * 2
@@ -796,6 +798,9 @@
     return stats
 
 
+MOMENTS = {"fused": os.environ.get("PCAA_MOMENTS_FUSED", "1") != "0"}
+
+
 def points_moments(x2d):
     _chk(x2d, "points_moments.x", torch.float32, 2)
     lib = _lib.load()
@@ -813,7 +818,15 @@
     _chk(x2d, "pointnet_in_moment_coeffs.x", torch.float32, 2)
     P, C = x2d.shape
     cout = W2d.shape[0]
-    if mom is None:
+    lib = _lib.load()
+    fused = mom is None and MOMENTS["fused"]
+    if fused:
+        n, nr = lib.pcaa_points_moments_size(), lib.pcaa_points_moments_rows_size(P)
+        buf = STATS_POOL.take_raw(n + nr + 2) if (STATS_POOL is not None and STATS_POOL.buf.device == x2d.device) else None
+        if buf is None:
+            buf = torch.zeros(n + nr + 2, dtype=torch.float64, device=x2d.device)
+        mom, rows, counter = buf[:n], buf[n:n + nr], buf[n + nr:n + nr + 1].view(torch.int32)
+    elif mom is None:
         mom = points_moments(x2d)
     tail = BnTailFwd(P, lin_bias, bn, cout, update_running=update_running)
     stats = mom
@@ -821,7 +834,11 @@
     tail.arm(stats)
     if not tail.armed:
         raise RuntimeError("pointnet_in_moment_coeffs: the carried finalize is switched off")
-    check(_lib.load().pcaa_pointnet_in_moment_stats(_p(mom), _p(W2d), C, cout, _s()), "pcaa_pointnet_in_moment_stats")
+    if fused:
+        check(lib.pcaa_points_moments_stats(_p(x2d), C, P, _p(mom), _p(rows), _p(counter), _p(W2d), cout, _s()),
+              "pcaa_points_moments_stats")
+    else:
+        check(lib.pcaa_pointnet_in_moment_stats(_p(mom), _p(W2d), C, cout, _s()), "pcaa_pointnet_in_moment_stats")
     TAILS["taken"] += 1
     return tail.out + (mom,)
 
@@ -1484,7 +1501,18 @@
     return da
 
 
-def chamfer(preds, gts, want_grad, grad_scale=1.0, grad_per_b=None):
+CHAMFER = {"variant": int(os.environ.get("PCAA_CHAMFER_FAST", "1")), "counters": {}}
+
+
+def _chamfer_counter(device):
+    key = torch.device(device)
+    c = CHAMFER["counters"].get(key)
+    if c is None:
+        c = CHAMFER["counters"][key] = torch.zeros(4, dtype=torch.int32, device=device)
+    return c
+
+
+def chamfer(preds, gts, want_grad, grad_scale=1.0, grad_per_b=None, total_scale=None, total_out=None, counter=None):
     for t, nm in ((preds, "preds"), (gts, "gts")):
         if not t.is_cuda or t.dtype != torch.float32 or t.dim() != 4:
             raise RuntimeError(f"chamfer: {nm} must be a 4-D float32 tensor on the HIP device")
@@ -1495,10 +1523,21 @@
     dp = torch.empty((B, C, T, N), dtype=torch.float32, device=preds.device) if want_grad else None
     ds = dp.stride() if want_grad else (0, 0, 0, 0)
     ps, gs = preds.stride(), gts.stride()
-    check(_lib.load().pcaa_chamfer_fwd_bwd(_p(preds), ps[0], ps[1], ps[2], ps[3], _p(gts), gs[0], gs[1], gs[2], gs[3],
-                                           B, T, N, C, _p(fl), _p(dp), ds[0], ds[1], ds[2], ds[3],
-                                           float(grad_scale), _p(grad_per_b), _s()), "pcaa_chamfer_fwd_bwd")
-    return fl, dp
+    tot = None
+    if total_scale is not None:
+        tot = torch.empty((), dtype=torch.float32, device=preds.device) if total_out is None else _chk(
+            total_out, "chamfer.total_out", torch.float32)
+        if tot.numel() != 1:
+            raise ValueError("chamfer: total_out must hold one float")
+        if counter is None:
+            counter = _chamfer_counter(preds.device)
+        elif not counter.is_cuda or counter.dtype != torch.int32 or counter.numel() < 1:
+            raise RuntimeError("chamfer: counter must be an int32 tensor on the HIP device")
+    check(_lib.load().pcaa_chamfer_fwd_bwd_total(
+        _p(preds), ps[0], ps[1], ps[2], ps[3], _p(gts), gs[0], gs[1], gs[2], gs[3], B, T, N, C, _p(fl), _p(dp),
+        ds[0], ds[1], ds[2], ds[3], float(grad_scale), _p(grad_per_b), float(total_scale or 0.0), _p(tot),
+        _p(counter) if tot is not None else None, CHAMFER["variant"], _s()), "pcaa_chamfer_fwd_bwd")
+    return (fl, dp) if total_scale is None else (fl, dp, tot)
 
 
 def cross_entropy(logits, target=None, want_loss=True, want_grad=False, grad_scale=1.0, want_preds=False,
@@ -1678,6 +1717,37 @@
         raise ValueError("adam_advance_: step_dev is int32[1], coef_dev float32[2]")
     check(_lib.load().pcaa_adam_advance(_p(step_dev), _p(coef_dev), float(lr), float(b1), float(b2), _s()),
           "pcaa_adam_advance")
+
+
+def step_begin_(zero0, zero1, count_a, count_b, lr, b1, b2):
+    ptrs = []
+    for z in (zero0, zero1):
+        if z is None or z.numel() == 0:
+            ptrs += [None, 0]
+            continue
+        if not z.is_cuda or not z.is_contiguous() or z.element_size() % 4 or z.data_ptr() % 16:
+            raise RuntimeError("step_begin_: regions are contiguous device tensors of 4- or 8-byte elements, 16-B aligned")
+        ptrs += [z.data_ptr(), z.numel() * z.element_size()]
+    cnt = []
+    for c in (count_a, count_b):
+        if c is None:
+            cnt += [None, None]
+            continue
+        _chk(c.step_dev, "step_begin.step_dev", torch.int32)
+        _chk(c.coef_dev, "step_begin.coef_dev", torch.float32)
+        if c.step_dev.numel() != 1 or c.coef_dev.numel() != 2:
+            raise ValueError("step_begin_: step_dev is int32[1], coef_dev float32[2]")
+        cnt += [c.step_dev.data_ptr(), c.coef_dev.data_ptr()]
+    check(_lib.load().pcaa_step_begin(*ptrs, *cnt, float(lr), float(b1), float(b2), _s()), "pcaa_step_begin")
+
+
+def sum3(a, b, c=None, out=None):
+    for t, nm in ((a, "a"), (b, "b"), (c, "c")):
+        if t is not None and (_chk(t, "sum3." + nm, torch.float32).numel() != 1):
+            raise ValueError("sum3: one-element tensors")
+    out = torch.empty((), dtype=torch.float32, device=a.device) if out is None else _chk(out, "sum3.out", torch.float32)
+    check(_lib.load().pcaa_sum3(_p(a), _p(b), _p(c), _p(out), _s()), "pcaa_sum3")
+    return out
 
 
 def adam_step_dev_(p, g, m, v, b1, b2, eps, coef_dev, grad_scale=1.0, max_blocks=0):
@@ -1814,6 +1884,8 @@
         rc = fwd(*operands, *shape, *split, _p(win_row.dev), win_row.segments, win_row.ring_rows, _s())
     check(rc, "pcaa_dtc_conv_fwd")
     if ksplit > 1 and stats is not None:
+        if tail is not None:
+            tail.arm(stats)
         check(lib.pcaa_splitk_reduce_stats(_p(dst), ksplit, stride, _p(y), _p(stats), NREP, rows, cout, _s()),
               "pcaa_splitk_reduce_stats")
     elif ksplit > 1:
diff --git a/opensetgaitrecognition_pcaa_amd/train.py b/opensetgaitrecognition_pcaa_amd/train.py
--- a/opensetgaitrecognition_pcaa_amd/train.py
+++ b/opensetgaitrecognition_pcaa_amd/train.py
@@ -21,6 +21,7 @@
 
 
 _SIDE_ADAM_AT = os.environ.get("PCAA_SIDE_ADAM_AT", "dec_bwd")
+_STEP_HELPERS = os.environ.get("PCAA_STEP_HELPERS", "1") != "0"
 
 
 def _side_streams(device):
@@ -334,6 +335,9 @@
             self._dec_grads16 = {i: (lo, self._g16[lo:lo + Wv.numel()].view(Wv.shape))
                                  for i, (lo, hi, Wv, mv, vv) in self._dec_fused.items()}
         self._stats_pool = ops.StatsPool(self.device)
+        self._gout_cache = {}
+        self.fused_helpers = _STEP_HELPERS
+        self._g_advanced = False
         self._flat_ready = True
         if self.pg is not None and self.world > 1:
             self.sync_replicas()
@@ -403,7 +407,34 @@
     def _collective(self):
         return self._xchg is not None and (self.world > 1 or self._force_collectives)
 
+    def _adv_gout(self, B, adv):
+        t = self._gout_cache.get((B, adv))
+        if t is None:
+            t = torch.full((B,), -adv / B, dtype=torch.float32, device=self.device)
+            if not torch.cuda.is_current_stream_capturing():
+                self._gout_cache[(B, adv)] = t
+        return t
+
+    def _begin_step(self, supervise):
+        self._g_advanced = False
+        if not self.fused_helpers:
+            self._stats_pool.begin()
+            self._enc_region.zero_()
+            return
+        fg = self.flat_g
+        b1, b2 = self.betas_g()
+        ops.step_begin_(self._stats_pool.begin(zero=False), self._enc_region, fg.count, fg.sup_count if supervise else None,
+                        self.cfg["LR"], b1, b2)
+        fg.count.step += 1
+        if supervise:
+            fg.sup_count.step += 1
+        else:
+            self._sup_split = True
+        self._g_advanced = True
+
     def _advance_g(self, supervise):
+        if self._g_advanced:
+            return
         b1, b2 = self.betas_g()
         self.flat_g.advance(self.cfg["LR"], b1, b2)
         if supervise:
@@ -473,8 +504,7 @@
         enc, dec = self.encoder, self.decoder
         gs = 1.0 / self.world
         ops.set_stats_pool(self._stats_pool)
-        self._stats_pool.begin()
-        self._enc_region.zero_()
+        self._begin_step(supervise)
         self.comm = {"collectives": 0, "payload_bytes": 0}
         F_hip._SYNC_BN["collectives"] = F_hip._SYNC_BN["payload_bytes"] = 0
         step_events = self._step_events = [] if self.time_comm else None
@@ -511,7 +541,7 @@
             self.flat_d.adam(cfg["LR"], cfg["B1"], cfg["B2"], grad_scale=gs)
             synth = ops.disc_forward(sup_fv, oh, self._d_params)
             lg = ops.total(synth, -adv / B, out=outs[1])
-            gout = torch.full((B,), -adv / B, dtype=torch.float32, device=self.device)
+            gout = self._adv_gout(B, adv)
             ds, _, _ = ops.disc_backward(sup_fv, oh, self._d_params, gout, want_dx=True, want_params=False, dx_out=outs[2])
             return dl, lg, ds
 
@@ -555,8 +585,13 @@
         F_hip.mark("dec_fwd")
         rec4 = rec.view(B, self.C, self.T, self.N)
         inv_bt = 1.0 / (B * self.T)
-        frame_loss, drec = ops.chamfer(rec4, pcs, want_grad=True, grad_scale=inv_bt)
-        rec_loss = ops.total(frame_loss, inv_bt)
+        if self.fused_helpers:
+            cnt = self._stats_pool.take_raw(2)
+            frame_loss, drec, rec_loss = ops.chamfer(rec4, pcs, want_grad=True, grad_scale=inv_bt, total_scale=inv_bt,
+                                                     counter=None if cnt is None else cnt.view(torch.int32))
+        else:
+            frame_loss, drec = ops.chamfer(rec4, pcs, want_grad=True, grad_scale=inv_bt)
+            rec_loss = ops.total(frame_loss, inv_bt)
 
         F_hip.mark("chamfer")
         F_hip.set_wgrad_stream(self._wg)
@@ -827,7 +862,10 @@
         F_hip.mark("adam+join")
         self.comm["collectives"] += F_hip._SYNC_BN.get("collectives", 0)
         self.comm["payload_bytes"] += F_hip._SYNC_BN.get("payload_bytes", 0)
-        tot = rec_loss + loss_g + (sup_loss if supervise else 0.0)
+        if self.fused_helpers:
+            tot = ops.sum3(rec_loss, loss_g, sup_loss if supervise else None)
+        else:
+            tot = rec_loss + loss_g + (sup_loss if supervise else 0.0)
         return {"d_loss": d_losses[0], "gp": d_losses[1], "rec_loss": rec_loss, "loss_g": loss_g,
                 "sup_loss": sup_loss, "tot_loss": tot, "preds": preds, "out_labels": logits, "sup_fvs": sup_fv}
 
@@ -891,8 +929,8 @@
             hproj = F_hip.linear_act_forward(sup_fv, self.decoder_projection_head[0], ACT_ELU)
         rec, _ = F_hip.decoder_forward(self.decoder, hproj, mode)
         B = pcs.shape[0]
-        fl, _ = ops.chamfer(rec.view(B, self.C, self.T, self.N), pcs, want_grad=False)
-        rec_loss = ops.total(fl, 1.0 / (B * self.T))
+        fl, _, rec_loss = ops.chamfer(rec.view(B, self.C, self.T, self.N), pcs, want_grad=False,
+                                      total_scale=1.0 / (B * self.T))
         ce, _, preds = ops.cross_entropy(logits, gt, want_loss=True, want_preds=True, err_flag=self._err)
         return rec_loss, ce, preds, sup_fv
 
```

Result: no change. 12310 sequences/s, median of 2 (-0.2%).
